# VitorMPCastro/MessyerRaytracer

Hardware: AMD Instinct MI355X
Metric: Mrays/s (primary, closest-hit) (higher is better)
Workload: dtype f32

## Files before the change

### messyerraytracer_amd/csrc/kernels.hip

```cpp
#include <hip/hip_runtime.h>
#include <cfloat>
#include <cstdarg>
#include <cstdio>
#include <cstdlib>
#include <type_traits>
#include "mrt_internal.h"

namespace mrt {

#define MRT_WG 256
#define MRT_WAVE 64

__device__ __forceinline__ float fma_(float a, float b, float c) { return __builtin_fmaf(a, b, c); }
__device__ __forceinline__ float dot3(float ax, float ay, float az, float bx, float by, float bz)
{
	return fma_(ax, bx, fma_(ay, by, az * bz));
}
__device__ __forceinline__ float safe_inv(float d)
{
	const float eps = 1e-9f;
	const float big = 1.0f / eps;
	return __builtin_fabsf(d) > eps ? 1.0f / d : (d >= 0.0f ? big : -big);
}

struct RayRegs {
	float ox, oy, oz, dx, dy, dz, t_min, t_max;
};

__device__ __forceinline__ bool skip_launch(const TraceParams &p)
{
	return p.skip_flag != nullptr && *p.skip_flag == p.skip_when;
}

__device__ __forceinline__ bool lane_ray_index_g(const TraceParams &p, uint64_t g, uint64_t &ray_idx, uint32_t &px, uint32_t &py);
__device__ __forceinline__ bool lane_ray_index(const TraceParams &p, uint32_t block, uint64_t &ray_idx, uint32_t &px, uint32_t &py)
{
	return lane_ray_index_g(p, (uint64_t)block * MRT_WG + threadIdx.x, ray_idx, px, py);
}
__device__ __forceinline__ bool xcd_strips(const TraceParams &p, uint64_t tile, uint32_t tiles_x, uint32_t tiles_y, uint32_t &tx, uint32_t &ty)
{
	const uint32_t tg = p.tile_group ? p.tile_group : 1u;
	uint32_t m = (tiles_x + 128u) >> 8;
	if (m == 0u) m = 1u;
	const uint32_t S = tiles_x / (8u * m);
	if (S == 0u || S * 8u * m != tiles_x || S % tg != 0u) return false;
	const uint64_t wg = tile / tg;
	const uint32_t k = (uint32_t)wg & 7u;
	const uint64_t j = (wg >> 3) * tg + tile % tg;
	const uint64_t per_strip = (uint64_t)S * tiles_y;
	const uint32_t sl = (uint32_t)(j / per_strip), r = (uint32_t)(j % per_strip);
	ty = r / S;
	tx = (sl * 8u + k) * S + r % S;
	return true;
}

__device__ __forceinline__ bool lane_ray_index_g(const TraceParams &p, uint64_t g, uint64_t &ray_idx, uint32_t &px, uint32_t &py)
{
	uint32_t lane_map = p.lane_map, grid_w = p.grid_w, rows = p.rows, tiles_x = p.tiles_x;
	if (lane_map == MAP_AUTO) {
		const uint32_t w = p.auto_grid[0];
		lane_map = w ? MAP_TILE8X8 : MAP_LINEAR;
		grid_w = w; rows = p.auto_grid[1]; tiles_x = p.auto_grid[2];
	}
	if (lane_map == MAP_TILE8X8) {
		uint64_t tile = g >> 6;
		const uint32_t l = (uint32_t)g & 63u;
		uint32_t tx, ty;
		const uint32_t k = p.tile_w_log2;
		const uint32_t tiles_y = (rows + (64u >> k) - 1u) >> (6u - k);
		uint32_t quarter = 4u;
		uint32_t sixteenth = 16u;
		if (p.quarter_all == 2u) { sixteenth = (uint32_t)tile & 15u; tile >>= 4; if (l >= 4u || tile >= (uint64_t)tiles_x * tiles_y) return false; }
		else if (p.quarter_all) { quarter = (uint32_t)tile & 3u; tile >>= 2; if (l >= 16u || tile >= (uint64_t)tiles_x * tiles_y) return false; }
		else if (p.tile_sched != nullptr && ((uint64_t)tiles_x * tiles_y + p.tile_unit - 1u) / p.tile_unit == p.n_units) {
			const uint64_t slot = tile / p.tile_unit;
			if (slot >= (p.sched_hdr ? p.sched_hdr[2] : p.n_units)) return false;
			const uint32_t e = p.tile_sched[slot], what = e >> 28, id = e & 0x0FFFFFFFu;
			if (what == 0u) tile = (uint64_t)id * p.tile_unit + tile % p.tile_unit;
			else {
				if (tile % p.tile_unit != 0u) return false;
				tile = id;
				if (what >= 2u) { quarter = what - 2u; if (l >= 16u) return false; }
			}
		}
		if (p.tile_order == 1u && (tiles_x & 15u) == 0u && (tiles_y & 15u) == 0u) {
			const uint32_t st = (uint32_t)(tile >> 8), in = (uint32_t)tile & 255u;
			uint32_t mx = in & 0x55u, my = (in >> 1) & 0x55u;
			mx = (mx | (mx >> 1)) & 0x33u; mx = (mx | (mx >> 2)) & 0x0Fu;
			my = (my | (my >> 1)) & 0x33u; my = (my | (my >> 2)) & 0x0Fu;
			const uint32_t stx = st % (tiles_x >> 4), sty = st / (tiles_x >> 4);
			tx = (stx << 4) + mx; ty = (sty << 4) + my;
		} else if (p.tile_order == 2u && (tiles_x & 31u) == 0u && (tiles_y & 31u) == 0u) {
			const uint32_t st = (uint32_t)(tile >> 10), in = (uint32_t)tile & 1023u;
			uint32_t mx = in & 0x155u, my = (in >> 1) & 0x155u;
			mx = (mx | (mx >> 1)) & 0x133u; mx = (mx | (mx >> 2)) & 0x10Fu; mx = (mx | (mx >> 4)) & 0x1Fu;
			my = (my | (my >> 1)) & 0x133u; my = (my | (my >> 2)) & 0x10Fu; my = (my | (my >> 4)) & 0x1Fu;
			const uint32_t stx = st % (tiles_x >> 5), sty = st / (tiles_x >> 5);
			tx = (stx << 5) + mx; ty = (sty << 5) + my;
		} else if (p.tile_order == 3u && xcd_strips(p, tile, tiles_x, tiles_y, tx, ty)) {
		} else { tx = (uint32_t)(tile % tiles_x); ty = (uint32_t)(tile / tiles_x); }
		if (sixteenth < 16u) {
			px = (tx << 3) + ((sixteenth & 3u) << 1) + (l & 1u);
			py = (ty << 3) + ((sixteenth >> 2) << 1) + (l >> 1);
		} else if (quarter < 4u) {
			px = (tx << 3) + ((quarter & 1u) << 2) + (l & 3u);
			py = (ty << 3) + ((quarter >> 1) << 2) + (l >> 2);
		} else {
			px = (tx << k) + (l & ((1u << k) - 1u));
			py = (ty << (6u - k)) + (l >> k);
		}
		if (px >= grid_w || py >= rows) return false;
		ray_idx = (uint64_t)py * grid_w + px;
		return true;
	}
	if (p.sparse_lanes) { const uint32_t l = (uint32_t)g & 63u; if (l >= p.sparse_lanes) return false; g = (g >> 6) * p.sparse_lanes + l; }
	if (g >= p.count) return false;
	ray_idx = p.perm ? (uint64_t)p.perm[g] : g;
	if (p.in_fmt == IN_GRID) { px = (uint32_t)(ray_idx % p.grid_w); py = (uint32_t)(ray_idx / p.grid_w); }
	return true;
}

__device__ __forceinline__ bool tile_cost_word(const TraceParams &p, uint64_t g_first, uint32_t *&park, uint32_t *&sum, uint32_t &what)
{
	if (p.tile_cost == nullptr) return false;
	uint32_t rows = p.rows, tiles_x = p.tiles_x;
	if (p.lane_map == MAP_AUTO) { if (p.auto_grid[0] == 0u) return false; rows = p.auto_grid[1]; tiles_x = p.auto_grid[2]; }
	else if (p.lane_map != MAP_TILE8X8) return false;
	const uint32_t k = p.tile_w_log2, tiles_y = (rows + (64u >> k) - 1u) >> (6u - k);
	if (((uint64_t)tiles_x * tiles_y + p.tile_unit - 1u) / p.tile_unit != p.n_units) return false;
	const uint64_t slot = (g_first >> 6) / p.tile_unit;
	what = 0u;
	if (p.tile_sched == nullptr) { if (slot >= p.n_units) return false; park = sum = p.tile_cost + slot; return true; }
	if (slot >= (p.sched_hdr ? p.sched_hdr[2] : p.n_units)) return false;
	const uint32_t e = p.tile_sched[slot], id = e & 0x0FFFFFFFu;
	what = e >> 28;
	if (what == 0u) { park = sum = p.tile_cost + id; return true; }
	park = p.tile_cost + p.n_units + slot;
	sum = p.tile_cost + id / p.tile_unit;
	return true;
}
__device__ __forceinline__ void note_tile_start(const TraceParams &p, uint64_t g_first)
{
	uint32_t *park, *sum, what;
	if (tile_cost_word(p, g_first, park, sum, what)) *park = (uint32_t)__builtin_amdgcn_s_memtime();
}
__device__ __forceinline__ void note_tile_cost(const TraceParams &p, uint64_t g_first)
{
	uint32_t *park, *sum, what;
	if (!tile_cost_word(p, g_first, park, sum, what)) return;
	uint32_t d = (uint32_t)__builtin_amdgcn_s_memtime() - *park;
	if (park == sum) { *sum = d ? d : 1u; return; }
	if (what == 1u) d = d - (d >> 2);
	else d = p.tile_unit == 2u ? (d >> 1) + (d >> 3) + (d >> 4) : d - (d >> 3);
	atomicAdd(sum, d ? d : 1u);
}

__device__ __forceinline__ void grid_ray(const TraceParams &p, uint32_t px, uint32_t py, RayRegs &r)
{
	const mrt_camera &c = p.cam;
	float dx, dy, dz;
	r.ox = c.origin[0]; r.oy = c.origin[1]; r.oz = c.origin[2];
	if (c.kind == MRT_CAMERA_DEBUG_GRID) {
		const float u = (2.0f * ((float)px + 0.5f) / (float)p.grid_w - 1.0f) * c.half_w;
		const float v = (2.0f * ((float)(py + p.y0) + 0.5f) / (float)p.grid_h - 1.0f) * c.half_h;
		dx = c.fwd[0] + c.right[0] * u + c.up[0] * v;
		dy = c.fwd[1] + c.right[1] * u + c.up[1] * v;
		dz = c.fwd[2] + c.right[2] * u + c.up[2] * v;
	} else {
		const float u = (2.0f * ((float)px + c.jitter_x) * c.inv_w) - 1.0f;
		const float v = 1.0f - (2.0f * ((float)(py + p.y0) + c.jitter_y) * c.inv_h);
		if (c.kind == MRT_CAMERA_PERSPECTIVE) {
			const float vx = u * c.half_w, vy = v * c.half_h;
			dx = c.right[0] * vx + c.up[0] * vy + c.fwd[0] * -1.0f;
			dy = c.right[1] * vx + c.up[1] * vy + c.fwd[1] * -1.0f;
			dz = c.right[2] * vx + c.up[2] * vy + c.fwd[2] * -1.0f;
		} else {
			const float sv = v * c.half_h, su = u * c.half_w;
			r.ox = (c.origin[0] + c.up[0] * sv) + c.right[0] * su;
			r.oy = (c.origin[1] + c.up[1] * sv) + c.right[1] * su;
			r.oz = (c.origin[2] + c.up[2] * sv) + c.right[2] * su;
			r.dx = -c.fwd[0]; r.dy = -c.fwd[1]; r.dz = -c.fwd[2];
			r.t_min = c.t_min; r.t_max = c.t_max;
			return;
		}
	}
	const float l2 = dx * dx + dy * dy + dz * dz;
	if (l2 == 0.0f) { dx = dy = dz = 0.0f; }
	else { const float l = __builtin_sqrtf(l2); dx /= l; dy /= l; dz /= l; }
	r.dx = dx; r.dy = dy; r.dz = dz;
	r.t_min = c.t_min; r.t_max = c.t_max;
}

__device__ __forceinline__ void load_ray(const TraceParams &p, uint64_t idx, uint32_t px, uint32_t py, RayRegs &r)
{
	if (p.in_fmt == IN_GRID) { grid_ray(p, px, py, r); return; }
	float ox, oy, oz, dx, dy, dz, t0, t1;
	if (p.in_fmt == IN_HOST60) {
		const float *h = reinterpret_cast<const float *>(p.rays) + idx * 15u;
		ox = h[0]; oy = h[1]; oz = h[2]; dx = h[3]; dy = h[4]; dz = h[5];
		t0 = h[12]; t1 = h[13];
	} else {
		const float4 *q = reinterpret_cast<const float4 *>(p.rays) + idx * 2u;
		const float4 a = q[0], b = q[1];
		ox = a.x; oy = a.y; oz = a.z; t1 = a.w;
		dx = b.x; dy = b.y; dz = b.z; t0 = b.w;
	}
	r.ox = ox; r.oy = oy; r.oz = oz; r.dx = dx; r.dy = dy; r.dz = dz; r.t_min = t0; r.t_max = t1;
}

__device__ __forceinline__ void store_hit(const TraceParams &p, uint64_t idx, const RayRegs &r,
		float t, int32_t prim, float u, float v, float nx, float ny, float nz, uint32_t layers, uint32_t slot)
{
	if (p.out_fmt == OUT_BOOL8) { reinterpret_cast<uint8_t *>(p.hits)[idx] = prim >= 0 ? 1 : 0; return; }
	if (p.out_fmt == OUT_TOKEN4) { reinterpret_cast<uint32_t *>(p.hits)[idx] = prim >= 0 ? slot : 0xFFFFFFFFu; return; }
	if (p.out_fmt == OUT_HOST44) {
		float *h = reinterpret_cast<float *>(p.hits) + idx * 11u;
		uint32_t *hu = reinterpret_cast<uint32_t *>(h);
		if (prim >= 0) {
			h[0] = t;
			h[1] = r.ox + r.dx * t; h[2] = r.oy + r.dy * t; h[3] = r.oz + r.dz * t;
			h[4] = nx; h[5] = ny; h[6] = nz; h[7] = u; h[8] = v;
			hu[9] = (uint32_t)prim; hu[10] = layers;
		} else {
			h[0] = FLT_MAX; h[1] = h[2] = h[3] = 0.0f; h[4] = h[5] = h[6] = 0.0f; h[7] = h[8] = 0.0f;
			hu[9] = 0xFFFFFFFFu; hu[10] = 0u;
		}
		return;
	}
	float4 *q = reinterpret_cast<float4 *>(p.hits) + idx * 2u;
	float4 a, b;
	a.x = t; a.y = __int_as_float(prim); a.z = u; a.w = v;
	b.x = nx; b.y = ny; b.z = nz; b.w = __uint_as_float(layers);
	q[0] = a; q[1] = b;
}

__device__ __forceinline__ void finish_ray(const TraceParams &p, uint64_t ray_idx, const RayRegs &r,
		float best_t, float best_u, float best_v, uint32_t best_slot)
{
	int32_t prim = -1; float nx = 0.0f, ny = 0.0f, nz = 0.0f; uint32_t layers = 0u;
	if (best_slot != 0xFFFFFFFFu) {
		if (p.out_fmt == OUT_BOOL8 || p.out_fmt == OUT_TOKEN4) prim = 0;
		else {
			prim = (int32_t)p.tri_hot[best_slot].id;
			layers = p.tri_hot[best_slot].layers;
			const float4 nn = reinterpret_cast<const float4 *>(p.tri_cold)[best_slot];
			nx = nn.x; ny = nn.y; nz = nn.z;
		}
	}
	store_hit(p, ray_idx, r, best_t, prim, best_u, best_v, nx, ny, nz, layers, best_slot);
}

__device__ __forceinline__ void finish_two_level_ray(const TraceParams &p, uint64_t ray_idx, const RayRegs &r,
		float best_t, float best_u, float best_v, uint32_t best_slot, uint32_t best_id, uint32_t best_inst)
{
	int32_t prim = -1; float nx = 0.0f, ny = 0.0f, nz = 0.0f; uint32_t layers = 0u;
	if (p.out_fmt == OUT_TOKEN8) {
		reinterpret_cast<uint2 *>(p.hits)[ray_idx] = make_uint2(best_slot, best_slot != 0xFFFFFFFFu ? best_inst : 0u);
		return;
	}
	if (best_slot != 0xFFFFFFFFu) {
		prim = (int32_t)best_id;
		if (p.out_fmt != OUT_BOOL8) {
			const float4 *row = reinterpret_cast<const float4 *>(p.instances) + (size_t)best_inst * 8u;
			const float4 b0 = row[3], b1 = row[4], b2 = row[5];
			const float4 no = reinterpret_cast<const float4 *>(p.tri_cold)[best_slot];
			nx = fma_(b0.x, no.x, fma_(b0.y, no.y, b0.z * no.z));
			ny = fma_(b0.w, no.x, fma_(b1.x, no.y, b1.y * no.z));
			nz = fma_(b1.z, no.x, fma_(b1.w, no.y, b2.x * no.z));
			const float l2 = fma_(nx, nx, fma_(ny, ny, nz * nz));
			if (l2 == 0.0f) { nx = ny = nz = 0.0f; }
			else { const float l = __builtin_sqrtf(l2); nx /= l; ny /= l; nz /= l; }
			layers = __float_as_uint(b2.w);
		}
	}
	store_hit(p, ray_idx, r, best_t, prim, best_u, best_v, nx, ny, nz, layers, best_slot);
}

#include "source_common.h"
#include "shadow_kernel.h"
#include "reflection_kernel.h"
#include "hemisphere_kernel.h"
#include "bounce_kernel.h"

template <bool ANY_HIT, bool COUNT>
__global__ __launch_bounds__(MRT_WG) void trace_lane_kernel(const TraceParams p)
{
	constexpr int SRC = SRC_CAST;
	const NoSource s{};
#include "lane_walk.inc"
}

#include "lane_persistent_kernel.h"
#include "packet_kernel.h"
#include "packet_asm_kernel.h"
#include "packet_rows_kernel.h"
#ifdef MRT_WITH_QUAD
#include "packet_quad_kernel.h"
#endif
#include "two_level_kernel.h"

template <class S, int SRC, bool ANY_HIT>
__global__ __launch_bounds__(MRT_WG) void trace_source_lane_kernel(const TraceParams p, const S s)
{
	constexpr bool COUNT = false;
#include "lane_walk.inc"
}
template <class S, int SRC, bool ANY_HIT>
__global__ __launch_bounds__(MRT_WG) void trace_source_two_level_kernel(const TraceParams p, const S s)
{
#include "two_level_walk.inc"
}
template <class S, int SRC, bool ANY_HIT, int WIDTH, bool TL>
__global__ __launch_bounds__(MRT_WG) MRT_PERSIST_ATTR void trace_source_persistent_kernel(const TraceParams p, const PersistParams q, const S s)
{
	constexpr bool COUNT = false;
#include "persistent_walk.inc"
}

__global__ __launch_bounds__(MRT_WG) void build_rows_kernel(const DevNode *nodes, const TriHot *hot, const TriCold *cold,
		uint32_t n_nodes, uint32_t n_tris, float4 *rows)
{
	const uint64_t g = (uint64_t)blockIdx.x * MRT_WG + threadIdx.x;
	if (g >= (uint64_t)n_nodes + n_tris) return;
	float4 *out = rows + g * 4u;
	if (g < n_nodes) {
		const float4 *n = reinterpret_cast<const float4 *>(nodes) + g * 4u;
		float4 a = n[0], b = n[1];
		uint32_t l = __float_as_uint(a.w), r = __float_as_uint(b.w);
		if (l >= kLeafBit) l = kLeafBit | (n_nodes + (l & 0x7FFFFFFFu));
		if (r >= kLeafBit) r = kLeafBit | (n_nodes + (r & 0x7FFFFFFFu));
		a.w = __uint_as_float(l); b.w = __uint_as_float(r);
		out[0] = a; out[1] = b; out[2] = n[2]; out[3] = n[3];
	} else {
		const uint64_t s = g - n_nodes;
		const float4 *t = reinterpret_cast<const float4 *>(hot) + s * 3u;
		out[0] = t[0]; out[1] = t[1]; out[2] = t[2];
		out[3] = reinterpret_cast<const float4 *>(cold)[s];
	}
}

hipError_t launch_build_rows(const DevNode *nodes, const TriHot *hot, const TriCold *cold, uint32_t n_nodes, uint32_t n_tris,
		void *rows, hipStream_t stream)
{
	const uint64_t total = (uint64_t)n_nodes + n_tris;
	hipLaunchKernelGGL(build_rows_kernel, dim3((uint32_t)((total + MRT_WG - 1) / MRT_WG)), dim3(MRT_WG), 0, stream,
			nodes, hot, cold, n_nodes, n_tris, reinterpret_cast<float4 *>(rows));
	return hipGetLastError();
}

__global__ __launch_bounds__(MRT_WG) void build_rows4_kernel(const Dev4Node *nodes4, const TriHot *hot, const TriCold *cold,
		uint32_t n_nodes4, uint32_t n_tris, float4 *rows)
{
	const uint64_t g = (uint64_t)blockIdx.x * MRT_WG + threadIdx.x;
	if (g >= (uint64_t)n_nodes4 + n_tris) return;
	if (g < n_nodes4) {
		const Dev4Node &n = nodes4[g];
		float *out = reinterpret_cast<float *>(rows + g * 8u);
		for (int k = 0; k < 4; k++)
			for (int c = 0; c < 3; c++) { out[6 * k + 2 * c] = n.box[k][c]; out[6 * k + 2 * c + 1] = n.box[k][3 + c]; }
		uint32_t *oref = reinterpret_cast<uint32_t *>(out) + 24;
		for (int i = 0; i < 4; i++) {
			const uint32_t ref = n.ref[i];
			oref[i] = ref == kSentinel ? ref : (ref >= kLeafBit ? (kLeafBit | (2u * n_nodes4 + (ref & 0x7FFFFFFFu))) : 2u * ref);
		}
		oref[4] = n.n_children; oref[5] = 0u; oref[6] = 0u; oref[7] = 0u;
	} else {
		const uint64_t s = g - n_nodes4;
		float4 *out = rows + ((uint64_t)2u * n_nodes4 + s) * 4u;
		const float4 *t = reinterpret_cast<const float4 *>(hot) + s * 3u;
		out[0] = t[0]; out[1] = t[1]; out[2] = t[2];
		out[3] = reinterpret_cast<const float4 *>(cold)[s];
	}
}

hipError_t launch_build_rows4(const Dev4Node *nodes4, const TriHot *hot, const TriCold *cold, uint32_t n_nodes4, uint32_t n_tris,
		void *rows, hipStream_t stream)
{
	const uint64_t total = (uint64_t)n_nodes4 + n_tris;
	hipLaunchKernelGGL(build_rows4_kernel, dim3((uint32_t)((total + MRT_WG - 1) / MRT_WG)), dim3(MRT_WG), 0, stream,
			nodes4, hot, cold, n_nodes4, n_tris, reinterpret_cast<float4 *>(rows));
	return hipGetLastError();
}

__global__ __launch_bounds__(MRT_WG) void grid_rays_kernel(const TraceParams p, mrt_ray32 *out)
{
	const uint64_t g = (uint64_t)blockIdx.x * MRT_WG + threadIdx.x;
	if (g >= p.count) return;
	RayRegs r;
	grid_ray(p, (uint32_t)(g % p.grid_w), (uint32_t)(g / p.grid_w), r);
	float4 *q = reinterpret_cast<float4 *>(out) + g * 2u;
	float4 a, b;
	a.x = r.ox; a.y = r.oy; a.z = r.oz; a.w = r.t_max;
	b.x = r.dx; b.y = r.dy; b.z = r.dz; b.w = r.t_min;
	q[0] = a; q[1] = b;
}

__global__ __launch_bounds__(MRT_WG) void expand_tokens_kernel(const TraceParams p, const uint32_t *tokens)
{
	const uint64_t g = (uint64_t)blockIdx.x * MRT_WG + threadIdx.x;
	if (g >= p.count) return;
	RayRegs r;
	uint32_t px = 0, py = 0;
	if (p.in_fmt == IN_GRID) { px = (uint32_t)(g % p.grid_w); py = (uint32_t)(g / p.grid_w); }
	load_ray(p, g, px, py, r);
	const uint32_t slot = tokens[g];
	if (slot >= p.n_tris) {
		store_hit(p, g, r, r.t_max, -1, 0.0f, 0.0f, 0.0f, 0.0f, 0.0f, 0u, slot);
		return;
	}
	const float4 *t3 = reinterpret_cast<const float4 *>(p.tri_hot) + (size_t)slot * 3u;
	const float4 q0 = t3[0], q1 = t3[1], q2 = t3[2];
	const float pvx = fma_(r.dy, q2.z, -(r.dz * q2.y));
	const float pvy = fma_(r.dz, q2.x, -(r.dx * q2.z));
	const float pvz = fma_(r.dx, q2.y, -(r.dy * q2.x));
	const float det = dot3(q1.x, q1.y, q1.z, pvx, pvy, pvz);
	const float inv_det = 1.0f / det;
	const float tvx = r.ox - q0.x, tvy = r.oy - q0.y, tvz = r.oz - q0.z;
	const float u = dot3(tvx, tvy, tvz, pvx, pvy, pvz) * inv_det;
	const float qvx = fma_(tvy, q1.z, -(tvz * q1.y));
	const float qvy = fma_(tvz, q1.x, -(tvx * q1.z));
	const float qvz = fma_(tvx, q1.y, -(tvy * q1.x));
	const float v = dot3(r.dx, r.dy, r.dz, qvx, qvy, qvz) * inv_det;
	const float t = dot3(q2.x, q2.y, q2.z, qvx, qvy, qvz) * inv_det;
	const float4 nn = reinterpret_cast<const float4 *>(p.tri_cold)[slot];
	store_hit(p, g, r, t, (int32_t)__float_as_uint(q0.w), u, v, nn.x, nn.y, nn.z, __float_as_uint(q1.w), slot);
}

__global__ __launch_bounds__(MRT_WG) void expand_two_level_tokens_kernel(const TraceParams p, const uint2 *tokens)
{
	const uint64_t g = (uint64_t)blockIdx.x * MRT_WG + threadIdx.x;
	if (g >= p.count) return;
	RayRegs r;
	uint32_t px = 0, py = 0;
	if (p.in_fmt == IN_GRID) { px = (uint32_t)(g % p.grid_w); py = (uint32_t)(g / p.grid_w); }
	load_ray(p, g, px, py, r);
	const uint2 tok = tokens[g];
	const uint32_t slot = tok.x, inst = tok.y;
	if (slot >= p.n_tris || inst >= p.n_instances) {
		finish_two_level_ray(p, g, r, r.t_max, 0.0f, 0.0f, 0xFFFFFFFFu, 0xFFFFFFFFu, 0u);
		return;
	}
	const float4 *row = reinterpret_cast<const float4 *>(p.instances) + (size_t)inst * 8u;
	const float4 m0 = row[0], m1 = row[1], m2 = row[2], meta = row[5];
	const float ox = fma_(m0.x, r.ox, fma_(m0.y, r.oy, fma_(m0.z, r.oz, m0.w)));
	const float oy = fma_(m1.x, r.ox, fma_(m1.y, r.oy, fma_(m1.z, r.oz, m1.w)));
	const float oz = fma_(m2.x, r.ox, fma_(m2.y, r.oy, fma_(m2.z, r.oz, m2.w)));
	const float dx = fma_(m0.x, r.dx, fma_(m0.y, r.dy, m0.z * r.dz));
	const float dy = fma_(m1.x, r.dx, fma_(m1.y, r.dy, m1.z * r.dz));
	const float dz = fma_(m2.x, r.dx, fma_(m2.y, r.dy, m2.z * r.dz));
	const float4 *t3 = reinterpret_cast<const float4 *>(p.tri_hot) + (size_t)slot * 3u;
	const float4 q0 = t3[0], q1 = t3[1], q2 = t3[2];
	const float pvx = fma_(dy, q2.z, -(dz * q2.y));
	const float pvy = fma_(dz, q2.x, -(dx * q2.z));
	const float pvz = fma_(dx, q2.y, -(dy * q2.x));
	const float det = dot3(q1.x, q1.y, q1.z, pvx, pvy, pvz);
	const float inv_det = 1.0f / det;
	const float tvx = ox - q0.x, tvy = oy - q0.y, tvz = oz - q0.z;
	const float u = dot3(tvx, tvy, tvz, pvx, pvy, pvz) * inv_det;
	const float qvx = fma_(tvy, q1.z, -(tvz * q1.y));
	const float qvy = fma_(tvz, q1.x, -(tvx * q1.z));
	const float qvz = fma_(tvx, q1.y, -(tvy * q1.x));
	const float v = dot3(dx, dy, dz, qvx, qvy, qvz) * inv_det;
	const float t = dot3(q2.x, q2.y, q2.z, qvx, qvy, qvz) * inv_det;
	finish_two_level_ray(p, g, r, t, u, v, slot, __float_as_uint(meta.z) + __float_as_uint(q0.w), inst);
}

#define MRT_DETECT_THREADS 1024
#define MRT_DETECT_MAX_RAYS 65536u
__device__ __forceinline__ void ray_dir(const void *rays, uint32_t in_fmt, uint64_t i, float &x, float &y, float &z)
{
	if (in_fmt == IN_HOST60) {
		const float *h = reinterpret_cast<const float *>(rays) + i * 15u;
		x = h[3]; y = h[4]; z = h[5];
	} else {
		const float4 b = reinterpret_cast<const float4 *>(rays)[i * 2u + 1u];
		x = b.x; y = b.y; z = b.z;
	}
}
__global__ __launch_bounds__(MRT_DETECT_THREADS) void detect_grid_kernel(const void *rays, uint32_t in_fmt, uint64_t count,
		uint32_t tile_w_log2, unsigned long long *scratch, uint32_t *out, uint32_t *host_out)
{
	__shared__ uint32_t first, second, is_last;
	const uint32_t m = (uint32_t)(count < (uint64_t)MRT_DETECT_MAX_RAYS ? count : (uint64_t)MRT_DETECT_MAX_RAYS);
	float ax, ay, az, bx, by, bz;
	ray_dir(rays, in_fmt, 0, ax, ay, az);
	ray_dir(rays, in_fmt, 1, bx, by, bz);
	const float step2 = (bx - ax) * (bx - ax) + (by - ay) * (by - ay) + (bz - az) * (bz - az);
	const float thr = 36.0f * step2;
	const uint32_t i = blockIdx.x * MRT_DETECT_THREADS + threadIdx.x;
	bool jump = false, wide = false;
	if (i >= 1 && i < m) {
		ray_dir(rays, in_fmt, i - 1, ax, ay, az);
		ray_dir(rays, in_fmt, i, bx, by, bz);
		const float d2 = (bx - ax) * (bx - ax) + (by - ay) * (by - ay) + (bz - az) * (bz - az);
		jump = d2 > thr;
		wide = !(d2 <= 0.01f);
	}
	const unsigned long long mask = __ballot(jump);
	const unsigned long long wmask_dir = __ballot(wide);
	if ((threadIdx.x & 63u) == 0u) {
		__hip_atomic_store(&scratch[i >> 6], mask, __ATOMIC_RELAXED, __HIP_MEMORY_SCOPE_AGENT);
		if (wmask_dir) atomicAdd(&scratch[1025], (unsigned long long)__builtin_popcountll(wmask_dir));
	}
	__threadfence();
	__syncthreads();
	if (threadIdx.x == 0) {
		const unsigned long long t = atomicAdd(&scratch[1024], 1ull);
		is_last = (t == (unsigned long long)gridDim.x - 1ull) ? 1u : 0u;
		first = 0xFFFFFFFFu; second = 0xFFFFFFFFu;
	}
	__syncthreads();
	if (!is_last) return;
	__threadfence();
	const uint32_t words = (m + 63u) >> 6;
	unsigned long long wmask = 0ull;
	if (threadIdx.x < words) wmask = __hip_atomic_load(&scratch[threadIdx.x], __ATOMIC_RELAXED, __HIP_MEMORY_SCOPE_AGENT);
	if (wmask) atomicMin(&first, threadIdx.x * 64u + (uint32_t)__builtin_ctzll(wmask));
	__syncthreads();
	const uint32_t f = first;
	if (f != 0xFFFFFFFFu && threadIdx.x >= (f >> 6)) {
		unsigned long long rest = wmask;
		if (threadIdx.x == (f >> 6)) rest &= ~((2ull << (f & 63u)) - 1ull);
		if (rest) atomicMin(&second, threadIdx.x * 64u + (uint32_t)__builtin_ctzll(rest));
	}
	__syncthreads();
	if (threadIdx.x == 0) {
		uint32_t w = first, rows = 0, tiles_x = 0;
		const uint32_t tw = 1u << tile_w_log2, th = 64u >> tile_w_log2;
		bool ok = step2 > 0.0f && w != 0xFFFFFFFFu && w >= 16u && (w % tw) == 0u && (count % w) == 0ull;
		if (ok) {
			const uint64_t r = count / w;
			ok = r <= 0xFFFFFFFFull && (r % th) == 0ull && (2ull * w >= m || second == 2u * w);
			rows = (uint32_t)r; tiles_x = w >> tile_w_log2;
		}
		out[0] = ok ? w : 0u; out[1] = ok ? rows : 0u; out[2] = ok ? tiles_x : 0u;
		const unsigned long long n_wide = __hip_atomic_load(&scratch[1025], __ATOMIC_RELAXED, __HIP_MEMORY_SCOPE_AGENT);
		out[3] = (n_wide * 8ull > (unsigned long long)m || (!ok && count < 32768ull)) ? 1u : 0u;
		if (host_out) { host_out[0] = out[0]; host_out[1] = out[1]; host_out[2] = out[2]; host_out[3] = out[3]; }
		scratch[1024] = 0ull; scratch[1025] = 0ull;
	}
}

hipError_t launch_detect_grid(const void *rays, uint32_t in_fmt, uint64_t count, uint32_t tile_w_log2,
		unsigned long long *scratch, uint32_t *out, uint32_t *host_out, hipStream_t stream)
{
	const uint32_t m = (uint32_t)(count < (uint64_t)MRT_DETECT_MAX_RAYS ? count : (uint64_t)MRT_DETECT_MAX_RAYS);
	const uint32_t blocks = (m + MRT_DETECT_THREADS - 1) / MRT_DETECT_THREADS;
	hipLaunchKernelGGL(detect_grid_kernel, dim3(blocks), dim3(MRT_DETECT_THREADS), 0, stream, rays, in_fmt, count, tile_w_log2, scratch, out, host_out);
	return hipGetLastError();
}

__device__ __forceinline__ uint32_t spread10(uint32_t v)
{
	v &= 0x000003FFu;
	v = (v | (v << 16)) & 0x030000FFu;
	v = (v | (v << 8)) & 0x0300F00Fu;
	v = (v | (v << 4)) & 0x030C30C3u;
	v = (v | (v << 2)) & 0x09249249u;
	return v;
}
__device__ __forceinline__ uint32_t quant10(float v)
{
	float n = (v + 1.0f) * 0.5f;
	n = fmaxf(0.0f, fminf(1.0f, n));
	return (uint32_t)(n * 1023.0f);
}
__global__ __launch_bounds__(MRT_WG) void morton_keys_kernel(const void *rays, uint32_t in_fmt, uint64_t count,
		uint32_t *keys, uint32_t *index)
{
	const uint64_t g = (uint64_t)blockIdx.x * MRT_WG + threadIdx.x;
	if (g >= count) return;
	float dx, dy, dz;
	if (in_fmt == IN_HOST60) {
		const float *h = reinterpret_cast<const float *>(rays) + g * 15u;
		dx = h[3]; dy = h[4]; dz = h[5];
	} else {
		const float4 b = reinterpret_cast<const float4 *>(rays)[g * 2u + 1u];
		dx = b.x; dy = b.y; dz = b.z;
	}
	keys[g] = (spread10(quant10(dx)) << 2) | (spread10(quant10(dy)) << 1) | spread10(quant10(dz));
	if (index) index[g] = (uint32_t)g;
}

__global__ __launch_bounds__(MRT_WG) void origin_dir_keys_kernel(const void *rays, uint32_t in_fmt, uint64_t count,
		float bx, float by, float bz, float sx, float sy, float sz, uint32_t *keys, uint32_t *index)
{
	const uint64_t g = (uint64_t)blockIdx.x * MRT_WG + threadIdx.x;
	if (g >= count) return;
	float ox, oy, oz, dx, dy, dz;
	if (in_fmt == IN_HOST60) {
		const float *h = reinterpret_cast<const float *>(rays) + g * 15u;
		ox = h[0]; oy = h[1]; oz = h[2]; dx = h[3]; dy = h[4]; dz = h[5];
	} else {
		const float4 a = reinterpret_cast<const float4 *>(rays)[g * 2u], b = reinterpret_cast<const float4 *>(rays)[g * 2u + 1u];
		ox = a.x; oy = a.y; oz = a.z; dx = b.x; dy = b.y; dz = b.z;
	}
	auto q = [](float v, float lo, float scale, float top) {
		const float n = fmaxf(0.0f, fminf(top, (v - lo) * scale));
		return (uint32_t)n;
	};
	const uint32_t qx = q(ox, bx, sx, 63.0f), qy = q(oy, by, sy, 63.0f), qz = q(oz, bz, sz, 63.0f);
	const uint32_t ex = q(dx, -1.0f, 8.0f, 15.0f), ey = q(dy, -1.0f, 8.0f, 15.0f), ez = q(dz, -1.0f, 8.0f, 15.0f);
	const uint32_t ko = (spread10(qx) << 2) | (spread10(qy) << 1) | spread10(qz);
	const uint32_t kd = (spread10(ex) << 2) | (spread10(ey) << 1) | spread10(ez);
	keys[g] = (ko << 12) | kd;
	if (index) index[g] = (uint32_t)g;
}

hipError_t launch_origin_dir_keys(const void *rays, uint32_t in_fmt, uint64_t count, const float lo[3], const float hi[3],
		uint32_t *keys, uint32_t *index, hipStream_t stream)
{
	if (count == 0) return hipSuccess;
	const uint64_t blocks = (count + MRT_WG - 1) / MRT_WG;
	float s[3];
	for (int k = 0; k < 3; k++) { const float e = hi[k] - lo[k]; s[k] = e > 0.0f ? 64.0f / e : 0.0f; }
	hipLaunchKernelGGL(origin_dir_keys_kernel, dim3((uint32_t)blocks), dim3(MRT_WG), 0, stream, rays, in_fmt, count,
			lo[0], lo[1], lo[2], s[0], s[1], s[2], keys, index);
	return hipGetLastError();
}

bool quad_kernel_built()
{
#ifdef MRT_WITH_QUAD
	return true;
#else
	return false;
#endif
}
static thread_local char g_variant[96] = "";
const char *last_trace_variant() { return g_variant; }
static void note_variant(const char *fmt, ...)
{
	va_list ap; va_start(ap, fmt); vsnprintf(g_variant, sizeof(g_variant), fmt, ap); va_end(ap);
}
#define MRT_B(x) ((x) ? "true" : "false")
#ifndef MRT_ROWS_WG_LARGE
#define MRT_ROWS_WG_LARGE MRT_WG
#endif
constexpr uint32_t kPrefetchMaxWaves = kWaveSlots + kWaveSlots / 4u;
hipError_t launch_trace(const TraceParams &p_in, bool any_hit, bool count, hipStream_t stream)
{
	TraceParams p = p_in;
	p.tile_group = (p.kernel == MRT_KERNEL_PACKET_DUAL && p.row_array != nullptr) ? 2u * ((p.rows_wg == 64u ? 64u : (uint32_t)MRT_ROWS_WG_LARGE) / MRT_WAVE) : MRT_WG / MRT_WAVE;
	uint64_t threads;
	if (p.tile_sched != nullptr && p.sched_hdr != nullptr && p.n_slots_max != 0u) {
		threads = (uint64_t)p.n_slots_max * p.tile_unit * 64u;
		if (p.lane_map == MAP_AUTO && threads < p.count) threads = p.count;
	} else if (p.lane_map == MAP_TILE8X8) {
		const uint32_t th = 64u >> p.tile_w_log2;
		threads = (uint64_t)p.tiles_x * ((p.rows + th - 1u) / th) * 64u * (p.quarter_all == 2u ? 16u : (p.quarter_all ? 4u : 1u));
	} else if (p.lane_map == MAP_LINEAR && p.sparse_lanes) threads = (p.count + p.sparse_lanes - 1u) / p.sparse_lanes * 64u;
	else threads = p.count * ((p.lane_map == MAP_AUTO && p.quarter_all) ? (p.quarter_all == 2u ? 16u : 4u) : 1u);
	if (threads == 0) return hipSuccess;
	const uint64_t blocks = (threads + MRT_WG - 1) / MRT_WG;
	if (blocks > 0x7FFFFFFFull) return hipErrorInvalidValue;
	dim3 grid((uint32_t)blocks), wg(MRT_WG);
	if (p.kernel == MRT_KERNEL_TWO_LEVEL_PACKET) {
		if (any_hit) hipLaunchKernelGGL((trace_two_level_packet_kernel<true>), grid, wg, p.extra_lds, stream, p);
		else hipLaunchKernelGGL((trace_two_level_packet_kernel<false>), grid, wg, p.extra_lds, stream, p);
		note_variant("trace_two_level_packet_kernel<%s>", MRT_B(any_hit));
		return hipGetLastError();
	}
	if (p.kernel == MRT_KERNEL_TWO_LEVEL) {
		const size_t lds2 = (size_t)(MRT_WG / MRT_WAVE) * p.stack_depth * MRT_WAVE * sizeof(uint32_t);
		if (any_hit) hipLaunchKernelGGL((trace_two_level_kernel<true>), grid, wg, lds2, stream, p);
		else hipLaunchKernelGGL((trace_two_level_kernel<false>), grid, wg, lds2, stream, p);
		note_variant("trace_two_level_kernel<%s>", MRT_B(any_hit));
		return hipGetLastError();
	}
#ifdef MRT_WITH_QUAD
	if (p.kernel == MRT_KERNEL_PACKET_QUAD && p.row_array4 != nullptr) {
		const uint64_t rblocks = (threads + 2u * MRT_WG - 1) / (2u * MRT_WG);
		dim3 rgrid((uint32_t)rblocks);
		if (count) {
			if (any_hit) hipLaunchKernelGGL((trace_packet_quad_kernel<true, true>), rgrid, wg, p.extra_lds, stream, p);
			else hipLaunchKernelGGL((trace_packet_quad_kernel<false, true>), rgrid, wg, p.extra_lds, stream, p);
		} else if (any_hit) hipLaunchKernelGGL((trace_packet_quad_kernel<true, false>), rgrid, wg, p.extra_lds, stream, p);
		else hipLaunchKernelGGL((trace_packet_quad_kernel<false, false>), rgrid, wg, p.extra_lds, stream, p);
		note_variant("trace_packet_quad_kernel<%s, %s>", MRT_B(any_hit), MRT_B(count));
		return hipGetLastError();
	}
#endif
	if ((p.kernel == MRT_KERNEL_PACKET_DUAL || p.kernel == MRT_KERNEL_PACKET_ROWS) && p.row_array != nullptr) {
		const uint32_t packets = p.kernel == MRT_KERNEL_PACKET_DUAL ? 2u : 1u;
		const uint32_t rows_wg = packets == 2u && p.rows_wg == 64u ? 64u : (packets == 2u ? (uint32_t)MRT_ROWS_WG_LARGE : (uint32_t)MRT_WG);
		const uint64_t rblocks = (threads + packets * rows_wg - 1) / (packets * rows_wg);
		dim3 rgrid((uint32_t)rblocks), rwg(rows_wg);
#define MRT_LAUNCH_ROWS(A, C, N, W, F) hipLaunchKernelGGL((trace_packet_rows_kernel<A, C, N, W, F>), rgrid, rwg, p.extra_lds, stream, p)
#define MRT_LAUNCH_ROWS_AC(N, W, F)                                                                                    \
		do {                                                                                                        \
			if (count) { if (any_hit) MRT_LAUNCH_ROWS(true, true, N, W, F); else MRT_LAUNCH_ROWS(false, true, N, W, F); } \
			else { if (any_hit) MRT_LAUNCH_ROWS(true, false, N, W, F); else MRT_LAUNCH_ROWS(false, false, N, W, F); }   \
		} while (0)
		const bool cull = packets == 2u && (p.rows_cull == 1u || (p.rows_cull == 2u && p.in_fmt == IN_GRID));
		if (packets == 2u && rows_wg == 64u) { if (cull) MRT_LAUNCH_ROWS_AC(2, 64, true); else MRT_LAUNCH_ROWS_AC(2, 64, false); }
		else if (packets == 2u) { if (cull) MRT_LAUNCH_ROWS_AC(2, MRT_ROWS_WG_LARGE, true); else MRT_LAUNCH_ROWS_AC(2, MRT_ROWS_WG_LARGE, false); }
		else MRT_LAUNCH_ROWS_AC(1, MRT_WG, false);
#undef MRT_LAUNCH_ROWS_AC
#undef MRT_LAUNCH_ROWS
		note_variant("trace_packet_rows_kernel<%s, %s, %u, %u, %s>", MRT_B(any_hit), MRT_B(count), packets, rows_wg, MRT_B(cull));
		return hipGetLastError();
	}
	if ((p.kernel == MRT_KERNEL_PACKET_ASM || p.kernel == MRT_KERNEL_PACKET_DUAL || p.kernel == MRT_KERNEL_PACKET_ROWS || p.kernel == MRT_KERNEL_PACKET_QUAD) && p.n_nodes < kAsmNodeLimit) {
		if (count) {
			if (any_hit) hipLaunchKernelGGL((trace_packet_asm_kernel<true, true>), grid, wg, p.extra_lds, stream, p);
			else hipLaunchKernelGGL((trace_packet_asm_kernel<false, true>), grid, wg, p.extra_lds, stream, p);
		} else {
			uint64_t waves = p.tile_sched != nullptr && p.n_slots_max != 0u ? (p.n_units > kWaveSlots ? p.n_units : (p.n_slots_max < kWaveSlots ? p.n_slots_max : kWaveSlots)) : threads / MRT_WAVE;
			if (p.lane_map == MAP_AUTO && waves < (p.count + MRT_WAVE - 1u) / MRT_WAVE) waves = (p.count + MRT_WAVE - 1u) / MRT_WAVE;
			const bool kpf = waves <= kPrefetchMaxWaves;
			if (kpf) { if (any_hit) hipLaunchKernelGGL((trace_packet_asm_kernel<true, false, true>), grid, wg, p.extra_lds, stream, p);
				else hipLaunchKernelGGL((trace_packet_asm_kernel<false, false, true>), grid, wg, p.extra_lds, stream, p); }
			else if (any_hit) hipLaunchKernelGGL((trace_packet_asm_kernel<true>), grid, wg, p.extra_lds, stream, p);
			else hipLaunchKernelGGL((trace_packet_asm_kernel<false>), grid, wg, p.extra_lds, stream, p);
			if (kpf) { note_variant("trace_packet_asm_kernel<%s, false, true>", MRT_B(any_hit)); return hipGetLastError(); }
		}
		note_variant("trace_packet_asm_kernel<%s, %s>", MRT_B(any_hit), MRT_B(count));
		return hipGetLastError();
	}
	if (p.kernel == MRT_KERNEL_PACKET || p.kernel == MRT_KERNEL_PACKET_ASM || p.kernel == MRT_KERNEL_PACKET_DUAL || p.kernel == MRT_KERNEL_PACKET_ROWS || p.kernel == MRT_KERNEL_PACKET_QUAD) {
		if (any_hit) {
			if (count) hipLaunchKernelGGL((trace_packet_kernel<true, true>), grid, wg, 0, stream, p);
			else hipLaunchKernelGGL((trace_packet_kernel<true, false>), grid, wg, 0, stream, p);
		} else {
			if (count) hipLaunchKernelGGL((trace_packet_kernel<false, true>), grid, wg, 0, stream, p);
			else hipLaunchKernelGGL((trace_packet_kernel<false, false>), grid, wg, 0, stream, p);
		}
		note_variant("trace_packet_kernel<%s, %s>", MRT_B(any_hit), MRT_B(count));
		return hipGetLastError();
	}
	const size_t lds = (size_t)(MRT_WG / MRT_WAVE) * p.stack_depth * MRT_WAVE * sizeof(uint32_t);
	if (any_hit) {
		if (count) hipLaunchKernelGGL((trace_lane_kernel<true, true>), grid, wg, lds, stream, p);
		else hipLaunchKernelGGL((trace_lane_kernel<true, false>), grid, wg, lds, stream, p);
	} else {
		if (count) hipLaunchKernelGGL((trace_lane_kernel<false, true>), grid, wg, lds, stream, p);
		else hipLaunchKernelGGL((trace_lane_kernel<false, false>), grid, wg, lds, stream, p);
	}
	note_variant("trace_lane_kernel<%s, %s>", MRT_B(any_hit), MRT_B(count));
	return hipGetLastError();
}

static PersistParams persist_params(const TraceParams &p, unsigned long long *next_ray, uint32_t *overflow,
		uint32_t lds_depth, uint32_t refill, uint32_t leaf_wait, uint32_t blocks)
{
	PersistParams q;
	q.next_ray = next_ray; q.overflow = overflow; q.overflow_stride = blocks * MRT_WG;
	q.lds_depth = lds_depth; q.refill = refill; q.leaf_wait = leaf_wait ? leaf_wait : 1u;
	const uint64_t per_wave = p.count / ((uint64_t)blocks * (MRT_WG / MRT_WAVE)) / 32u;
	q.chunk = per_wave >= MRT_RAY_CHUNK ? MRT_RAY_CHUNK : (per_wave <= MRT_WAVE ? MRT_WAVE : (uint32_t)(per_wave & ~63ull));
	return q;
}

hipError_t launch_trace_persistent(const TraceParams &p, unsigned long long *next_ray, uint32_t *overflow,
		uint32_t lds_depth, uint32_t refill, uint32_t leaf_wait, uint32_t blocks, bool any_hit, bool count, hipStream_t stream)
{
	if (p.count == 0 || blocks == 0) return hipSuccess;
	const PersistParams q = persist_params(p, next_ray, overflow, lds_depth, refill, leaf_wait, blocks);
	const size_t lds = (size_t)(MRT_WG / MRT_WAVE) * lds_depth * MRT_WAVE * sizeof(uint32_t);
	const bool wide8 = p.kernel == MRT_KERNEL_LANE8_PERSISTENT && p.nodes8 != nullptr;
	const bool wide4 = p.kernel == MRT_KERNEL_LANE4_PERSISTENT && p.nodes4 != nullptr;
	if (p.kernel == MRT_KERNEL_TWO_LEVEL_PERSISTENT8 && p.nodes8 != nullptr && p.leaf_box != nullptr) {
		if (any_hit) hipLaunchKernelGGL((trace_lane_persistent_kernel<true, 8, true>), dim3(blocks), dim3(MRT_WG), lds, stream, p, q);
		else hipLaunchKernelGGL((trace_lane_persistent_kernel<false, 8, true>), dim3(blocks), dim3(MRT_WG), lds, stream, p, q);
	} else if (p.kernel == MRT_KERNEL_TWO_LEVEL_PERSISTENT || p.kernel == MRT_KERNEL_TWO_LEVEL_PERSISTENT8) {
		if (any_hit) hipLaunchKernelGGL((trace_lane_persistent_kernel<true, 2, true>), dim3(blocks), dim3(MRT_WG), lds, stream, p, q);
		else hipLaunchKernelGGL((trace_lane_persistent_kernel<false, 2, true>), dim3(blocks), dim3(MRT_WG), lds, stream, p, q);
	} else if (count) {
#define MRT_LP(A, W) hipLaunchKernelGGL((trace_lane_persistent_kernel<A, W, false, true>), dim3(blocks), dim3(MRT_WG), lds, stream, p, q)
		if (wide8) { if (any_hit) MRT_LP(true, 8); else MRT_LP(false, 8); }
		else if (wide4) { if (any_hit) MRT_LP(true, 4); else MRT_LP(false, 4); }
		else { if (any_hit) MRT_LP(true, 2); else MRT_LP(false, 2); }
#undef MRT_LP
	} else if (wide8) {
		if (any_hit) hipLaunchKernelGGL((trace_lane_persistent_kernel<true, 8>), dim3(blocks), dim3(MRT_WG), lds, stream, p, q);
		else hipLaunchKernelGGL((trace_lane_persistent_kernel<false, 8>), dim3(blocks), dim3(MRT_WG), lds, stream, p, q);
	} else if (wide4) {
		if (any_hit) hipLaunchKernelGGL((trace_lane_persistent_kernel<true, 4>), dim3(blocks), dim3(MRT_WG), lds, stream, p, q);
		else hipLaunchKernelGGL((trace_lane_persistent_kernel<false, 4>), dim3(blocks), dim3(MRT_WG), lds, stream, p, q);
	} else {
		if (any_hit) hipLaunchKernelGGL((trace_lane_persistent_kernel<true, 2>), dim3(blocks), dim3(MRT_WG), lds, stream, p, q);
		else hipLaunchKernelGGL((trace_lane_persistent_kernel<false, 2>), dim3(blocks), dim3(MRT_WG), lds, stream, p, q);
	}
	{
		const bool tl = p.kernel == MRT_KERNEL_TWO_LEVEL_PERSISTENT || p.kernel == MRT_KERNEL_TWO_LEVEL_PERSISTENT8;
		const int width = tl ? ((p.kernel == MRT_KERNEL_TWO_LEVEL_PERSISTENT8 && p.nodes8 != nullptr && p.leaf_box != nullptr) ? 8 : 2) : (wide8 ? 8 : (wide4 ? 4 : 2));
		note_variant("trace_lane_persistent_kernel<%s, %d, %s, %s>", MRT_B(any_hit), width, MRT_B(tl), MRT_B(count && !tl));
	}
	return hipGetLastError();
}

template <class S, int SRC, bool ANY_HIT>
static void launch_source_as(const TraceParams &p, const S &s, unsigned long long *next_ray, uint32_t *overflow,
		uint32_t lds_depth, uint32_t refill, uint32_t leaf_wait, uint32_t blocks, hipStream_t stream)
{
	using F = SourceFamily<S>;
	const bool tl = p.kernel == MRT_KERNEL_TWO_LEVEL || p.kernel == MRT_KERNEL_TWO_LEVEL_PERSISTENT || p.kernel == MRT_KERNEL_TWO_LEVEL_PERSISTENT8;
	char mode[8] = "";
	if (F::any_hit && F::nearest) snprintf(mode, sizeof(mode), ", %s", MRT_B(ANY_HIT));
	if (blocks == 0) {
		const uint64_t threads = p.sparse_lanes ? (p.count + p.sparse_lanes - 1u) / p.sparse_lanes * 64u : p.count;
		const dim3 grid((uint32_t)((threads + MRT_WG - 1) / MRT_WG)), wg(MRT_WG);
		const size_t lds = (size_t)(MRT_WG / MRT_WAVE) * p.stack_depth * MRT_WAVE * sizeof(uint32_t);
		if (tl) hipLaunchKernelGGL((trace_source_two_level_kernel<S, SRC, ANY_HIT>), grid, wg, lds, stream, p, s);
		else hipLaunchKernelGGL((trace_source_lane_kernel<S, SRC, ANY_HIT>), grid, wg, lds, stream, p, s);
		note_variant("trace_%s_%s_kernel<%d%s>", F::name, tl ? "two_level" : "lane", SRC, mode);
		return;
	}
	const PersistParams q = persist_params(p, next_ray, overflow, lds_depth, refill, leaf_wait, blocks);
	const size_t lds = (size_t)(MRT_WG / MRT_WAVE) * q.lds_depth * MRT_WAVE * sizeof(uint32_t);
#define MRT_LS(W, T) hipLaunchKernelGGL((trace_source_persistent_kernel<S, SRC, ANY_HIT, W, T>), dim3(blocks), dim3(MRT_WG), lds, stream, p, q, s)
	int width = 2;
	if (tl && p.kernel == MRT_KERNEL_TWO_LEVEL_PERSISTENT8 && p.nodes8 != nullptr && p.leaf_box != nullptr) { width = 8; MRT_LS(8, true); }
	else if (tl) MRT_LS(2, true);
	else if (p.kernel == MRT_KERNEL_LANE8_PERSISTENT && p.nodes8 != nullptr) { width = 8; MRT_LS(8, false); }
	else if (p.kernel == MRT_KERNEL_LANE4_PERSISTENT && p.nodes4 != nullptr) { width = 4; MRT_LS(4, false); }
	else MRT_LS(2, false);
#undef MRT_LS
	note_variant("trace_%s_persistent_kernel<%d%s, %d, %s>", F::name, SRC, mode, width, MRT_B(tl));
}

template <class S>
hipError_t launch_source(const TraceParams &p, const void *params, int src, bool any_hit, unsigned long long *next_ray, uint32_t *overflow,
		uint32_t lds_depth, uint32_t refill, uint32_t leaf_wait, uint32_t blocks, hipStream_t stream)
{
	using F = SourceFamily<S>;
	const S &s = *static_cast<const S *>(params);
	if (p.count == 0) return hipSuccess;
	const uint64_t threads = p.sparse_lanes ? (p.count + p.sparse_lanes - 1u) / p.sparse_lanes * 64u : p.count;
	if (blocks == 0 && (threads + MRT_WG - 1) / MRT_WG > 0x7FFFFFFFull) return hipErrorInvalidValue;
	if ((src != F::ray32 && src != F::host && src != F::grid) || !(any_hit ? F::any_hit : F::nearest)) return hipErrorInvalidValue;
#define MRT_LS_SRC(A)                                                                                                                        \
	do {                                                                                                                                 \
		if (src == F::ray32) launch_source_as<S, F::ray32, A>(p, s, next_ray, overflow, lds_depth, refill, leaf_wait, blocks, stream);   \
		else if (src == F::host) launch_source_as<S, F::host, A>(p, s, next_ray, overflow, lds_depth, refill, leaf_wait, blocks, stream); \
		else launch_source_as<S, F::grid, A>(p, s, next_ray, overflow, lds_depth, refill, leaf_wait, blocks, stream);                     \
	} while (0)
	if constexpr (F::any_hit) { if (any_hit) MRT_LS_SRC(true); }
	if constexpr (F::nearest) { if (!any_hit) MRT_LS_SRC(false); }
#undef MRT_LS_SRC
	return hipGetLastError();
}
template hipError_t launch_source<ShadowParams>(const TraceParams &, const void *, int, bool, unsigned long long *, uint32_t *, uint32_t, uint32_t, uint32_t, uint32_t, hipStream_t);
template hipError_t launch_source<ReflectParams>(const TraceParams &, const void *, int, bool, unsigned long long *, uint32_t *, uint32_t, uint32_t, uint32_t, uint32_t, hipStream_t);
template hipError_t launch_source<HemiParams>(const TraceParams &, const void *, int, bool, unsigned long long *, uint32_t *, uint32_t, uint32_t, uint32_t, uint32_t, hipStream_t);
template hipError_t launch_source<BounceParams>(const TraceParams &, const void *, int, bool, unsigned long long *, uint32_t *, uint32_t, uint32_t, uint32_t, uint32_t, hipStream_t);

hipError_t launch_grid_rays(const TraceParams &p, mrt_ray32 *out, hipStream_t stream)
{
	if (p.count == 0) return hipSuccess;
	const uint64_t blocks = (p.count + MRT_WG - 1) / MRT_WG;
	hipLaunchKernelGGL(grid_rays_kernel, dim3((uint32_t)blocks), dim3(MRT_WG), 0, stream, p, out);
	return hipGetLastError();
}

hipError_t launch_expand_tokens(const TraceParams &p, const uint32_t *tokens, hipStream_t stream)
{
	if (p.count == 0) return hipSuccess;
	const uint64_t blocks = (p.count + MRT_WG - 1) / MRT_WG;
	if (p.instances != nullptr)
		hipLaunchKernelGGL(expand_two_level_tokens_kernel, dim3((uint32_t)blocks), dim3(MRT_WG), 0, stream, p, reinterpret_cast<const uint2 *>(tokens));
	else hipLaunchKernelGGL(expand_tokens_kernel, dim3((uint32_t)blocks), dim3(MRT_WG), 0, stream, p, tokens);
	return hipGetLastError();
}

hipError_t launch_morton_keys(const void *rays, uint32_t in_fmt, uint64_t count, uint32_t *keys, uint32_t *index, hipStream_t stream)
{
	if (count == 0) return hipSuccess;
	const uint64_t blocks = (count + MRT_WG - 1) / MRT_WG;
	hipLaunchKernelGGL(morton_keys_kernel, dim3((uint32_t)blocks), dim3(MRT_WG), 0, stream, rays, in_fmt, count, keys, index);
	return hipGetLastError();
}

}
```

### messyerraytracer_amd/csrc/packet_rows_kernel.h

```cpp
#pragma once

#define RA_LMINX "s20"
#define RA_LMINY "s21"
#define RA_LMINZ "s22"
#define RA_LREF "s23"
#define RA_LMAXX "s24"
#define RA_LMAXY "s25"
#define RA_LMAXZ "s26"
#define RA_RREF "s27"
#define RA_RMINX "s28"
#define RA_RMINY "s29"
#define RA_RMINZ "s30"
#define RA_RMAXX "s32"
#define RA_RMAXY "s33"
#define RA_RMAXZ "s34"
#define RA_MASK "s[60:61]"
#define RA_MASKLO "s60"
#define RA_MASKHI "s61"
#define RA_V0X "s20"
#define RA_V0Y "s21"
#define RA_V0Z "s22"
#define RA_ID "s23"
#define RA_E1X "s24"
#define RA_E1Y "s25"
#define RA_E1Z "s26"
#define RA_LAYERS "s27"
#define RA_E2X "s28"
#define RA_E2Y "s29"
#define RA_E2Z "s30"
#define RA_FLAGS "s31"

#define MRT_NEAR_0(RS, AX, SIDE) RS##_##SIDE##MIN##AX
#define MRT_NEAR_1(RS, AX, SIDE) RS##_##SIDE##MAX##AX
#define MRT_FAR_0(RS, AX, SIDE) RS##_##SIDE##MAX##AX
#define MRT_FAR_1(RS, AX, SIDE) RS##_##SIDE##MIN##AX

#define MRT_OP(NAME, P) "%[" NAME P "]"

#define MRT_ROWS_SLAB(P, RS, BX, BY, BZ)                                                                             \
	"v_fma_f32 v50, " MRT_NEAR_##BX(RS, X, L) ", " MRT_OP("ix", P) ", " MRT_OP("nrx", P) "\n"                        \
	"v_fma_f32 v51, " MRT_NEAR_##BY(RS, Y, L) ", " MRT_OP("iy", P) ", " MRT_OP("nry", P) "\n"                        \
	"v_fma_f32 v52, " MRT_NEAR_##BZ(RS, Z, L) ", " MRT_OP("iz", P) ", " MRT_OP("nrz", P) "\n"                        \
	"v_fma_f32 v53, " MRT_FAR_##BX(RS, X, L) ", " MRT_OP("ix", P) ", " MRT_OP("nrx", P) "\n"                         \
	"v_fma_f32 v54, " MRT_FAR_##BY(RS, Y, L) ", " MRT_OP("iy", P) ", " MRT_OP("nry", P) "\n"                         \
	"v_fma_f32 v55, " MRT_FAR_##BZ(RS, Z, L) ", " MRT_OP("iz", P) ", " MRT_OP("nrz", P) "\n"                         \
	"v_max_f32 v52, v52, " MRT_OP("tmin", P) "\n"                                                                   \
	"v_fma_f32 v56, " MRT_NEAR_##BX(RS, X, R) ", " MRT_OP("ix", P) ", " MRT_OP("nrx", P) "\n"                        \
	"v_min_f32 v55, v55, " MRT_OP("lim", P) "\n"                                                                    \
	"v_fma_f32 v57, " MRT_NEAR_##BY(RS, Y, R) ", " MRT_OP("iy", P) ", " MRT_OP("nry", P) "\n"                        \
	"v_max3_f32 v50, v50, v51, v52\n"                                                               \
	"v_fma_f32 v51, " MRT_NEAR_##BZ(RS, Z, R) ", " MRT_OP("iz", P) ", " MRT_OP("nrz", P) "\n"                        \
	"v_min3_f32 v53, v53, v54, v55\n"                                                               \
	"v_fma_f32 v52, " MRT_FAR_##BX(RS, X, R) ", " MRT_OP("ix", P) ", " MRT_OP("nrx", P) "\n"                         \
	"v_fma_f32 v54, " MRT_FAR_##BY(RS, Y, R) ", " MRT_OP("iy", P) ", " MRT_OP("nry", P) "\n"                         \
	"v_fma_f32 v55, " MRT_FAR_##BZ(RS, Z, R) ", " MRT_OP("iz", P) ", " MRT_OP("nrz", P) "\n"                         \
	"v_max_f32 v51, v51, " MRT_OP("tmin", P) "\n"                                                                   \
	"v_min_f32 v55, v55, " MRT_OP("lim", P) "\n"                                                                    \
	"v_max3_f32 v56, v56, v57, v51\n"                                                               \
	"v_min3_f32 v52, v52, v54, v55\n"

#define MRT_ROWS_NODE_STEP(P, RS, POPBIT, CNT_P, BX, BY, BZ)                                                                 \
	MRT_ROWS_SLAB(P, RS, BX, BY, BZ)                                                                                \
	"v_cmp_le_f32 vcc, v50, v53\n"                                             \
	"v_cmp_le_f32_e64 s[54:55], v56, v52\n"                                    \
	"s_cbranch_vccz L_" P "lmiss_%=\n"                                                                              \
	"s_cmp_eq_u64 s[54:55], 0\n"                                                                                    \
	"s_cbranch_scc1 L_" P "onlyl_%=\n"                                                                              \
	"v_cmp_lt_f32_e64 s[56:57], v50, v56\n"     \
	"s_bitcmp1_b32 s56, 0\n"                                                                                        \
	"s_cselect_b32 s53, " RS##_RREF ", " RS##_LREF "\n"                                                    \
	"s_cselect_b32 " MRT_OP("cur", P) ", " RS##_LREF ", " RS##_RREF "\n"                                   \
	"s_cselect_b64 s[58:59], s[54:55], vcc\n"                                   \
	"s_cselect_b64 " RS##_MASK ", vcc, s[54:55]\n"                               \
	"v_mov_b32 v51, s53\n"                                                                                          \
	"v_mov_b32 v52, s58\n"                                                                                          \
	"v_mov_b32 v53, s59\n"                                                                                          \
	"ds_write_b32 " MRT_OP("sp", P) ", v51\n"                                                                       \
	"ds_write_b64 " MRT_OP("sp", P) ", v[52:53] offset:8\n"                                                         \
	"v_add_u32 " MRT_OP("sp", P) ", 16, " MRT_OP("sp", P) "\n"                                                      \
	CNT_P                                                                                                           \
	"v_lshlrev_b32 v54, 6, v51\n"             \
	"global_load_dword v60, v54, %[rows]\n"   \
	"s_branch L_" P "done_%=\n"                                                                                     \
	"L_" P "onlyl_%=:\n"                                                                                            \
	"s_mov_b32 " MRT_OP("cur", P) ", " RS##_LREF "\n"                                                                \
	"s_mov_b64 " RS##_MASK ", vcc\n"                                                                                 \
	"s_branch L_" P "done_%=\n"                                                                                     \
	"L_" P "lmiss_%=:\n"                                                                                            \
	"s_cmp_eq_u64 s[54:55], 0\n"                                                                                    \
	"s_cbranch_scc1 L_" P "npop_%=\n"                                                                               \
	"s_mov_b32 " MRT_OP("cur", P) ", " RS##_RREF "\n"                                                                \
	"s_mov_b64 " RS##_MASK ", s[54:55]\n"                                                                            \
	"s_branch L_" P "done_%=\n"                                                                                     \
	"L_" P "npop_%=:\n"                                                                                             \
	"s_or_b32 %[ev], %[ev], " POPBIT "\n"

#define MRT_ROWS_TRI_TEST(P, RS, OWNMASK, CUROP, ANYHIT_CODE)                                                        \
	"s_and_b32 s52, " RS##_LAYERS ", %[qmask]\n"                    \
	"s_cbranch_scc0 L_" P "tnext_%=\n"                                                                              \
	"v_mul_f32 v50, " RS##_E2Y ", " MRT_OP("dz", P) "\n"                                                             \
	"v_mul_f32 v51, " RS##_E2Z ", " MRT_OP("dx", P) "\n"                                                             \
	"v_mul_f32 v52, " RS##_E2X ", " MRT_OP("dy", P) "\n"                                                             \
	"v_fma_f32 v50, " MRT_OP("dy", P) ", " RS##_E2Z ", -v50\n"                            \
	"v_fma_f32 v51, " MRT_OP("dz", P) ", " RS##_E2X ", -v51\n"                            \
	"v_fma_f32 v52, " MRT_OP("dx", P) ", " RS##_E2Y ", -v52\n"                            \
	"v_mul_f32 v53, " RS##_E1Z ", v52\n"                                                                             \
	"v_fma_f32 v53, " RS##_E1Y ", v51, v53\n"                                                                        \
	"v_fma_f32 v53, " RS##_E1X ", v50, v53\n"                                                     \
	"v_cmp_nlt_f32_e64 s[54:55], |v53|, %[eps]\n"                                              \
	"s_and_b64 s[54:55], s[54:55], " OWNMASK "\n"                       \
	"s_cbranch_scc0 L_" P "tnext_%=\n"                                                                              \
	"v_div_scale_f32 v54, s[56:57], v53, v53, 1.0\n"                   \
	"v_rcp_f32 v55, v54\n"                                                                                          \
	"v_div_scale_f32 v56, vcc, 1.0, v53, 1.0\n"                                                                     \
	"v_subrev_f32 v59, " RS##_V0X ", " MRT_OP("ox", P) "\n"       \
	"v_fma_f32 v57, -v54, v55, 1.0\n"                                                                               \
	"v_fma_f32 v55, v57, v55, v55\n"                                                                                \
	"v_mul_f32 v57, v56, v55\n"                                                                                     \
	"v_fma_f32 v58, -v54, v57, v56\n"                                                                               \
	"v_fma_f32 v57, v58, v55, v57\n"                                                                                \
	"v_fma_f32 v54, -v54, v57, v56\n"                                                                               \
	"v_div_fmas_f32 v54, v54, v55, v57\n"                                                                           \
	"v_div_fixup_f32 v54, v54, v53, 1.0\n"                                                       \
	"v_subrev_f32 v55, " RS##_V0Y ", " MRT_OP("oy", P) "\n"                                                 \
	"v_subrev_f32 v56, " RS##_V0Z ", " MRT_OP("oz", P) "\n"                                                 \
	"v_mul_f32 v58, v56, v52\n"                                                                                     \
	"v_fma_f32 v58, v55, v51, v58\n"                                                                                \
	"v_fma_f32 v58, v59, v50, v58\n"                                                                                \
	"v_mul_f32 v58, v58, v54\n"                                                    \
	"v_cmp_nlt_f32_e64 s[56:57], v58, 0\n"                                                            \
	"v_cmp_ngt_f32_e64 s[58:59], v58, 1.0\n"                                                          \
	"s_and_b64 s[54:55], s[54:55], s[56:57]\n"                                                                      \
	"s_and_b64 s[54:55], s[54:55], s[58:59]\n"                                                                      \
	"s_cbranch_scc0 L_" P "tnext_%=\n"                                                                              \
	"v_mul_f32 v50, " RS##_E1Y ", v56\n"                                                                             \
	"v_mul_f32 v51, " RS##_E1Z ", v59\n"                                                                             \
	"v_mul_f32 v52, " RS##_E1X ", v55\n"                                                                             \
	"v_fma_f32 v50, v55, " RS##_E1Z ", -v50\n"                                          \
	"v_fma_f32 v51, v56, " RS##_E1X ", -v51\n"                                          \
	"v_fma_f32 v52, v59, " RS##_E1Y ", -v52\n"                                          \
	"v_mul_f32 v59, " MRT_OP("dz", P) ", v52\n"                                                                     \
	"v_fma_f32 v59, " MRT_OP("dy", P) ", v51, v59\n"                                                                \
	"v_fma_f32 v59, " MRT_OP("dx", P) ", v50, v59\n"                                                                \
	"v_mul_f32 v59, v59, v54\n"                                                     \
	"v_add_f32 v55, v58, v59\n"                                                                          \
	"v_cmp_nlt_f32_e64 s[56:57], v59, 0\n"                                                            \
	"v_cmp_ngt_f32_e64 s[58:59], v55, 1.0\n"                                                      \
	"s_and_b64 s[54:55], s[54:55], s[56:57]\n"                                                                      \
	"s_and_b64 s[54:55], s[54:55], s[58:59]\n"                                                                      \
	"s_cbranch_scc0 L_" P "tnext_%=\n"                                                                              \
	"v_mul_f32 v55, " RS##_E2Z ", v52\n"                                                                             \
	"v_fma_f32 v55, " RS##_E2Y ", v51, v55\n"                                                                        \
	"v_fma_f32 v55, " RS##_E2X ", v50, v55\n"                                                                        \
	"v_mul_f32 v55, v55, v54\n"                                                    \
	                          \
	"v_cmp_nlt_f32_e64 s[56:57], v55, " MRT_OP("tmin", P) "\n"                                                      \
	"v_cmp_lt_f32_e64 s[58:59], v55, " MRT_OP("lim", P) "\n"                                                        \
	"v_cmp_eq_f32_e64 s[64:65], v55, " MRT_OP("lim", P) "\n"                                                        \
	"v_cmp_ne_u32_e64 s[66:67], " MRT_OP("bs", P) ", -1\n"                                                          \
	"v_cmp_gt_u32_e64 vcc, " MRT_OP("bi", P) ", " RS##_ID "\n"                                     \
	"s_and_b64 s[64:65], s[64:65], s[66:67]\n"                                                                      \
	"s_and_b64 s[64:65], s[64:65], vcc\n"                                                                           \
	"s_or_b64 s[58:59], s[58:59], s[64:65]\n"                                                                       \
	"s_and_b64 s[54:55], s[54:55], s[56:57]\n"                                                                      \
	"s_and_b64 s[54:55], s[54:55], s[58:59]\n"                                    \
	"s_cbranch_scc0 L_" P "tnext_%=\n"                                                                              \
	"s_and_b32 s52, " CUROP ", 0x7fffffff\n"                                                \
	"v_mov_b32 v50, s52\n"                                                                                          \
	"v_mov_b32 v51, " RS##_ID "\n"                                                                                   \
	"v_cndmask_b32_e64 " MRT_OP("bt", P) ", " MRT_OP("bt", P) ", v55, s[54:55]\n"                                   \
	"v_cndmask_b32_e64 " MRT_OP("bu", P) ", " MRT_OP("bu", P) ", v58, s[54:55]\n"                                   \
	"v_cndmask_b32_e64 " MRT_OP("bv", P) ", " MRT_OP("bv", P) ", v59, s[54:55]\n"                                   \
	"v_cndmask_b32_e64 " MRT_OP("bs", P) ", " MRT_OP("bs", P) ", v50, s[54:55]\n"                                   \
	"v_cndmask_b32_e64 " MRT_OP("bi", P) ", " MRT_OP("bi", P) ", v51, s[54:55]\n"                                   \
	ANYHIT_CODE                                                                                                     \
	"L_" P "tnext_%=:\n"

#define MRT_ROWS_TRI_STEP(P, RS, POPBIT, CNT_T, ANYHIT_CODE)                                                         \
	CNT_T                                                                                                           \
	MRT_ROWS_TRI_TEST(P, RS, RS##_MASK, MRT_OP("cur", P), ANYHIT_CODE)                                              \
	"s_bitcmp1_b32 " RS##_FLAGS ", 0\n"                                          \
	"s_cbranch_scc1 L_" P "tpop_%=\n"                                                                               \
	"s_add_u32 " MRT_OP("cur", P) ", " MRT_OP("cur", P) ", 1\n"                                                     \
	"s_branch L_" P "done_%=\n"                                                                                     \
	"L_" P "tpop_%=:\n"                                                                                             \
	"s_or_b32 %[ev], %[ev], " POPBIT "\n"

#define MRT_ROWS_NEAREST(P) \
	"v_cndmask_b32_e64 " MRT_OP("lim", P) ", " MRT_OP("lim", P) ", v55, s[54:55]\n"
#define MRT_ROWS_ANYHIT(P, DONEBIT) \
	"v_cndmask_b32_e64 " MRT_OP("lim", P) ", " MRT_OP("lim", P) ", %[vneg], s[54:55]\n"                             \
	"v_cmp_neq_f32_e64 s[56:57], " MRT_OP("lim", P) ", %[vneg]\n"                                                   \
	"s_cmp_lg_u64 s[56:57], 0\n"                                                                                    \
	"s_cbranch_scc1 L_" P "tnext_%=\n"                                                                              \
	"s_mov_b32 " MRT_OP("cur", P) ", 0x7fffffff\n"                                                                  \
	"s_or_b32 %[ev], %[ev], " DONEBIT "\n"                                                                          \
	"s_branch L_" P "done_%=\n"

#define MRT_ROWS_STEP(P, RS, POPBIT, CNT_N, CNT_T, CNT_P, ANYHIT_CODE, BX, BY, BZ)                                            \
	"s_bitcmp1_b32 " MRT_OP("cur", P) ", 31\n"                                                                      \
	"s_cbranch_scc1 L_" P "tri_%=\n"                                                                                \
	CNT_N                                                                                                           \
	MRT_ROWS_NODE_STEP(P, RS, POPBIT, CNT_P, BX, BY, BZ)                                                             \
	"s_branch L_" P "done_%=\n"                                                                                     \
	"L_" P "tri_%=:\n"                                                                                              \
	MRT_ROWS_TRI_STEP(P, RS, POPBIT, CNT_T, ANYHIT_CODE)                                                             \
	"L_" P "done_%=:\n"

#define MRT_ROWS_POP_ISSUE(P, POPBITNO, V0123)                                                                      \
	"s_bitcmp1_b32 %[ev], " POPBITNO "\n"                                                                           \
	"s_cbranch_scc0 L_" P "pi_%=\n"                                                                                 \
	"v_add_u32 " MRT_OP("sp", P) ", -16, " MRT_OP("sp", P) "\n"                                                     \
	"ds_read_b128 " V0123 ", " MRT_OP("sp", P) "\n"                                                                 \
	"L_" P "pi_%=:\n"
#define MRT_ROWS_POP_TAKE(P, RS, POPBITNO, V0, V2, V3)                                                               \
	"s_bitcmp1_b32 %[ev], " POPBITNO "\n"                                                                           \
	"s_cbranch_scc0 L_" P "pt_%=\n"                                                                                 \
	"v_readfirstlane_b32 " MRT_OP("cur", P) ", " V0 "\n"                                                            \
	"v_readfirstlane_b32 " RS##_MASKLO ", " V2 "\n"                                                                  \
	"v_readfirstlane_b32 " RS##_MASKHI ", " V3 "\n"                                                                  \
	"L_" P "pt_%=:\n"

#define MRT_ROWS_CLOBBERS                                                                                             \
	"vcc", "scc", "s20", "s21", "s22", "s23", "s24", "s25", "s26", "s27", "s28", "s29", "s30", "s31", "s32", "s33", \
	"s34", "s35", "s36", "s37", "s38", "s39", "s40", "s41", "s42", "s43", "s44", "s45", "s46", "s47", "s48", "s49", \
	"s50", "s51", "s52", "s53", "s54", "s55", "s56", "s57", "s58", "s59", "s60", "s61", "s62", "s63", "s64", "s65", \
	"s66", "s67", "v50", "v51", "v52", "v53", "v54", "v55", "v56", "v57", "v58", "v59", "v60"

#define MRT_ROWS_OUT(P, S)                                                                                            \
	[cur##P] "+s"(S.cur), [sp##P] "+v"(S.sp), [lim##P] "+v"(S.lim), [bt##P] "+v"(S.bt), [bu##P] "+v"(S.bu),         \
	[bv##P] "+v"(S.bv), [bs##P] "+v"(S.bs), [bi##P] "+v"(S.bi), [mask##P] "+s"(S.mask)
#define MRT_ROWS_IN(P, S)                                                                                             \
	[ox##P] "v"(S.ox), [oy##P] "v"(S.oy), [oz##P] "v"(S.oz), [dx##P] "v"(S.dx), [dy##P] "v"(S.dy), [dz##P] "v"(S.dz), \
	[tmin##P] "v"(S.tmin), [ix##P] "v"(S.ix), [iy##P] "v"(S.iy), [iz##P] "v"(S.iz), [nrx##P] "v"(S.nrx),            \
	[nry##P] "v"(S.nry), [nrz##P] "v"(S.nrz)

struct PacketRegs {
	float ox, oy, oz, dx, dy, dz, tmin;
	float ix, iy, iz, nrx, nry, nrz;
	float lim;
	float bt, bu, bv;
	uint32_t bs, bi;
	uint32_t sp;
	uint32_t cur;
	unsigned long long mask;
};

#define MRT_ROWS_LOOP1(CNT_N, CNT_T, CNT_P, T_PRE, T_POST, ANYHIT_CODE, BX, BY, BZ)                                          \
	asm volatile(                                                                                                   \
		"s_mov_b64 s[60:61], %[maskA]\n"                                                                            \
		"L_loop_%=:\n"                                                                                              \
		"s_lshl_b32 s52, %[curA], 6\n"                                                                              \
		T_PRE                                                                                                       \
		"s_load_dwordx16 s[20:35], %[rows], s52\n"                                                                  \
		"s_waitcnt lgkmcnt(0)\n"                                                                                    \
		T_POST                                                                                                      \
		MRT_ROWS_STEP("A", RA, "1", CNT_N, CNT_T, CNT_P, ANYHIT_CODE, BX, BY, BZ)                                   \
		"s_cmp_eq_u32 %[ev], 0\n"                                                                                   \
		"s_cbranch_scc1 L_loop_%=\n"                                                                                \
		MRT_ROWS_POP_ISSUE("A", "0", "v[50:53]")                                                                    \
		"s_waitcnt lgkmcnt(0)\n"                                                                                    \
		MRT_ROWS_POP_TAKE("A", RA, "0", "v50", "v52", "v53")                                                        \
		"s_mov_b32 %[ev], 0\n"                                                                                      \
		"s_cmp_lg_u32 %[curA], 0x7fffffff\n"                                                                        \
		"s_cbranch_scc1 L_loop_%=\n"                                                                                \
		"s_waitcnt vmcnt(0)\n"                    \
		"s_mov_b64 %[maskA], s[60:61]\n"                                                                            \
		: MRT_ROWS_OUT(A, a), [ev] "+s"(ev), [cntn] "+s"(cnt_n), [cntt] "+s"(cnt_t), [cntw] "+s"(cnt_w), [cntp] "+s"(sp_max) \
		: MRT_ROWS_IN(A, a), [rows] "s"(rows), [qmask] "s"(qmask), [eps] "s"(eps), [vneg] "v"(vneg)                 \
		: MRT_ROWS_CLOBBERS)

#define MRT_ROWSW_GROUP_SLAB(P, OWN, LM, RM, BX, BY, BZ)                                                              \
	"s_cmp_eq_u64 " OWN ", 0\n"                                                                                     \
	"s_cbranch_scc1 L_" P "skip_%=\n"                             \
	MRT_ROWS_SLAB(P, RA, BX, BY, BZ)                                                                                \
	"v_cmp_le_f32_e64 " LM ", v50, v53\n"                                                                           \
	"v_cmp_le_f32_e64 " RM ", v56, v52\n"                                                                           \
	"L_" P "sdone_%=:\n"
#define MRT_ROWSW_GROUP_SKIP(P, LM, RM)                                                                               \
	"L_" P "skip_%=:\n"                                                                                             \
	"s_mov_b64 " LM ", 0\n"                                                                                         \
	"s_mov_b64 " RM ", 0\n"                                                                                         \
	"s_branch L_" P "sdone_%=\n"

#define MRT_ROWSW_ANYHIT(P) \
	"v_cndmask_b32_e64 " MRT_OP("lim", P) ", " MRT_OP("lim", P) ", %[vneg], s[54:55]\n"
#define MRT_ROWSW_ANYDONE                                                                                             \
	"v_cmp_neq_f32_e64 s[56:57], %[limA], %[vneg]\n"                                                                \
	"v_cmp_neq_f32_e64 s[58:59], %[limB], %[vneg]\n"                                                                \
	"s_or_b64 s[56:57], s[56:57], s[58:59]\n"                                                                       \
	"s_cbranch_scc1 L_goon_%=\n"                                                                                    \
	"s_mov_b32 %[curA], 0x7fffffff\n"                                                                               \
	"s_branch L_exit_%=\n"                                                                                          \
	"L_goon_%=:\n"

#ifndef MRT_ROWS_KPREFETCH
#define MRT_ROWS_KPREFETCH 1
#endif
#if MRT_ROWS_KPREFETCH
#define MRT_ROWSW_KPREFETCH                                                                                           \
	"s_lshl_b32 s48, " RA_LREF ", 6\n"                                                                               \
	"s_lshl_b32 s49, " RA_RREF ", 6\n"                                                                               \
	"s_load_dword s64, %[rows], s48\n"                                                                              \
	"s_load_dword s65, %[rows], s49\n"
#define MRT_ROWSW_FARPREFETCH ""
#else
#define MRT_ROWSW_KPREFETCH ""
#define MRT_ROWSW_FARPREFETCH                                                                                         \
	"v_lshlrev_b32 v55, 6, v54\n"                                       \
	"global_load_dword v60, v55, %[rows]\n"
#endif

#define MRT_ROWS_LOOPW(CNT_N, CNT_T, CNT_P, ANYA, ANYB, ANYDONE, BX, BY, BZ)                                                 \
	asm volatile(                                                                                                   \
		"s_mov_b64 s[60:61], %[maskA]\n"                                                                            \
		"s_mov_b64 s[62:63], %[maskB]\n"                                                                            \
		"L_loop_%=:\n"                                                                                              \
		"s_lshl_b32 s52, %[curA], 6\n"                                                                              \
		"s_load_dwordx16 s[20:35], %[rows], s52\n"                                                                  \
		"s_waitcnt lgkmcnt(0)\n"                                                                                    \
		"s_bitcmp1_b32 %[curA], 31\n"                                                                               \
		"s_cbranch_scc1 L_tri_%=\n"                                                                                 \
		CNT_N                                                                                                       \
		MRT_ROWSW_KPREFETCH                                                                                         \
		MRT_ROWSW_GROUP_SLAB("A", "s[60:61]", "s[36:37]", "s[38:39]", BX, BY, BZ)                                   \
		MRT_ROWSW_GROUP_SLAB("B", "s[62:63]", "s[40:41]", "s[42:43]", BX, BY, BZ)                                   \
		"s_or_b64 s[44:45], s[36:37], s[40:41]\n"                     \
		"s_cbranch_scc0 L_lmiss_%=\n"                                                                               \
		"s_or_b64 vcc, s[38:39], s[42:43]\n"                                              \
		"s_cbranch_scc0 L_onlyl_%=\n"                                                                               \
		      \
		"v_cmp_lt_f32_e64 s[46:47], v50, v56\n"                                           \
		"s_bitcmp1_b32 s46, 0\n"                                                                                    \
		"s_cselect_b32 s53, " RA_RREF ", " RA_LREF "\n"                                                   \
		"s_cselect_b32 %[curA], " RA_LREF ", " RA_RREF "\n"                                               \
		"s_cselect_b64 s[50:51], s[38:39], s[36:37]\n"                 \
		"s_cselect_b64 s[58:59], s[42:43], s[40:41]\n"                                                              \
		"s_cselect_b64 s[60:61], s[36:37], s[38:39]\n"                                        \
		"s_cselect_b64 s[62:63], s[40:41], s[42:43]\n"                                                              \
		"v_mov_b32 v50, s50\n"                                                                                      \
		"v_mov_b32 v51, s51\n"                                                                                      \
		"v_mov_b32 v52, s58\n"                                                                                      \
		"v_mov_b32 v53, s59\n"                                                                                      \
		"v_mov_b32 v54, s53\n"                                                                                      \
		"ds_write_b128 %[spA], v[50:53]\n"                                                                          \
		"ds_write_b32 %[spA], v54 offset:16\n"                                                                      \
		"v_add_u32 %[spA], 32, %[spA]\n"                                                                            \
		CNT_P                                                                                                       \
		MRT_ROWSW_FARPREFETCH                                                                                       \
		"s_branch L_loop_%=\n"                                                                                      \
		"L_onlyl_%=:\n"                                                                                             \
		"s_mov_b32 %[curA], " RA_LREF "\n"                                                                          \
		"s_mov_b64 s[60:61], s[36:37]\n"                                                                            \
		"s_mov_b64 s[62:63], s[40:41]\n"                                                                            \
		"s_branch L_loop_%=\n"                                                                                      \
		"L_lmiss_%=:\n"                                                                                             \
		"s_or_b64 vcc, s[38:39], s[42:43]\n"                                                                        \
		"s_cbranch_scc0 L_pop_%=\n"                                                                                 \
		"s_mov_b32 %[curA], " RA_RREF "\n"                                                                          \
		"s_mov_b64 s[60:61], s[38:39]\n"                                                                            \
		"s_mov_b64 s[62:63], s[42:43]\n"                                                                            \
		"s_branch L_loop_%=\n"                                                                                      \
		"L_tri_%=:\n"                                                                                               \
		CNT_T                                                                                                       \
		"s_cmp_eq_u64 s[60:61], 0\n"                                                                                \
		"s_cbranch_scc1 L_Atnext_%=\n"                                                                              \
		MRT_ROWS_TRI_TEST("A", RA, "s[60:61]", "%[curA]", ANYA)                                                     \
		"s_cmp_eq_u64 s[62:63], 0\n"                                                                                \
		"s_cbranch_scc1 L_Btnext_%=\n"                                                                              \
		MRT_ROWS_TRI_TEST("B", RA, "s[62:63]", "%[curA]", ANYB)                                                     \
		ANYDONE                                                                                                     \
		"s_bitcmp1_b32 " RA_FLAGS ", 0\n"                                       \
		"s_cbranch_scc1 L_pop_%=\n"                                                                                 \
		"s_add_u32 %[curA], %[curA], 1\n"                                                                           \
		"s_branch L_loop_%=\n"                                                                                      \
		"L_pop_%=:\n"                                                                                               \
		"v_add_u32 %[spA], -32, %[spA]\n"                                                                           \
		"ds_read_b128 v[50:53], %[spA]\n"                                                                           \
		"ds_read_b32 v54, %[spA] offset:16\n"                                                                       \
		"s_waitcnt lgkmcnt(0)\n"                                                                                    \
		"v_readfirstlane_b32 %[curA], v54\n"                                                                        \
		"v_readfirstlane_b32 s60, v50\n"                                                                            \
		"v_readfirstlane_b32 s61, v51\n"                                                                            \
		"v_readfirstlane_b32 s62, v52\n"                                                                            \
		"v_readfirstlane_b32 s63, v53\n"                                                                            \
		"s_cmp_lg_u32 %[curA], 0x7fffffff\n"                                                                        \
		"s_cbranch_scc1 L_loop_%=\n"                                                                                \
		"s_branch L_exit_%=\n"                                                                                      \
		MRT_ROWSW_GROUP_SKIP("A", "s[36:37]", "s[38:39]")                                                           \
		MRT_ROWSW_GROUP_SKIP("B", "s[40:41]", "s[42:43]")                                                           \
		"L_exit_%=:\n"                                                                                              \
		"s_waitcnt vmcnt(0)\n"                    \
		"s_mov_b64 %[maskA], s[60:61]\n"                                                                            \
		"s_mov_b64 %[maskB], s[62:63]\n"                                                                            \
		: MRT_ROWS_OUT(A, a), [limB] "+v"(b.lim), [btB] "+v"(b.bt), [buB] "+v"(b.bu), [bvB] "+v"(b.bv),             \
		  [bsB] "+v"(b.bs), [biB] "+v"(b.bi), [maskB] "+s"(b.mask), [cntn] "+s"(cnt_n), [cntt] "+s"(cnt_t), [cntp] "+s"(sp_max) \
		: MRT_ROWS_IN(A, a), MRT_ROWS_IN(B, b), [rows] "s"(rows), [qmask] "s"(qmask), [eps] "s"(eps), [vneg] "v"(vneg) \
		: MRT_ROWS_CLOBBERS)


#define MRT_ROWS_SLAB1(P, RS, SIDE, TE, BX, BY, BZ, MASK)                                                             \
	"v_fma_f32 v51, " MRT_NEAR_##BX(RS, X, SIDE) ", " MRT_OP("ix", P) ", " MRT_OP("nrx", P) "\n"                      \
	"v_fma_f32 v52, " MRT_NEAR_##BY(RS, Y, SIDE) ", " MRT_OP("iy", P) ", " MRT_OP("nry", P) "\n"                      \
	"v_fma_f32 v53, " MRT_NEAR_##BZ(RS, Z, SIDE) ", " MRT_OP("iz", P) ", " MRT_OP("nrz", P) "\n"                      \
	"v_fma_f32 v54, " MRT_FAR_##BX(RS, X, SIDE) ", " MRT_OP("ix", P) ", " MRT_OP("nrx", P) "\n"                       \
	"v_fma_f32 v55, " MRT_FAR_##BY(RS, Y, SIDE) ", " MRT_OP("iy", P) ", " MRT_OP("nry", P) "\n"                       \
	"v_fma_f32 v57, " MRT_FAR_##BZ(RS, Z, SIDE) ", " MRT_OP("iz", P) ", " MRT_OP("nrz", P) "\n"                       \
	"v_max_f32 v53, v53, " MRT_OP("tmin", P) "\n"                                                                   \
	"v_min_f32 v57, v57, " MRT_OP("lim", P) "\n"                                                                    \
	"v_max3_f32 " TE ", v51, v52, v53\n"                                                                            \
	"v_min3_f32 v54, v54, v55, v57\n"                                                                               \
	"v_cmp_le_f32_e64 " MASK ", " TE ", v54\n"

#define MRT_ROWSC_CHILD(SIDE, TE, CULLBITS, MA, MB, BX, BY, BZ)                                                       \
	"s_and_b32 s48, s44, " CULLBITS "\n"                                 \
	"s_cbranch_scc1 L_cull" #SIDE "_%=\n"                                                                           \
	"s_cmp_eq_u64 s[60:61], 0\n"                                                                                    \
	"s_cbranch_scc1 L_" #SIDE "A0_%=\n"                                                                             \
	MRT_ROWS_SLAB1("A", RA, SIDE, TE, BX, BY, BZ, MA)                                                               \
	"L_" #SIDE "A1_%=:\n"                                                                                           \
	"s_cmp_eq_u64 s[62:63], 0\n"                                                                                    \
	"s_cbranch_scc1 L_" #SIDE "B0_%=\n"                                                                             \
	MRT_ROWS_SLAB1("B", RA, SIDE, TE, BX, BY, BZ, MB)                                                               \
	"L_" #SIDE "B1_%=:\n"
#define MRT_ROWSC_CHILD_OOL(SIDE, MA, MB)                                                                             \
	"L_cull" #SIDE "_%=:\n"                                                                                         \
	MRT_ROWSC_CNT_CULL                                                                                              \
	"s_mov_b64 " MA ", 0\n"                                                                                         \
	"s_mov_b64 " MB ", 0\n"                                                                                         \
	"s_branch L_" #SIDE "B1_%=\n"                                                                                   \
	"L_" #SIDE "A0_%=:\n"                                                                                           \
	"s_mov_b64 " MA ", 0\n"                                                                                         \
	"s_branch L_" #SIDE "A1_%=\n"                                                                                   \
	"L_" #SIDE "B0_%=:\n"                                                                                           \
	"s_mov_b64 " MB ", 0\n"                                                                                         \
	"s_branch L_" #SIDE "B1_%=\n"
#define MRT_ROWSC_CNT_CULL ""

#define MRT_ROWSC_VLOAD(VDST, REF)                                                                                   \
	"v_lshl_add_u32 v62, " REF ", 6, %[cvo]\n"                                                                      \
	"global_load_dword " VDST ", v62, %[rows]\n"

#ifndef MRT_ROWSC_KPF
#define MRT_ROWSC_KPF 0
#endif
#if MRT_ROWSC_KPF
#define MRT_ROWSC_KPREFETCH                                                                                           \
	"s_lshl_b32 s46, " RA_LREF ", 6\n"                                                                               \
	"s_lshl_b32 s47, " RA_RREF ", 6\n"                                                                               \
	"s_load_dword s64, %[rows], s46\n"                                                                              \
	"s_load_dword s65, %[rows], s47\n"
#else
#define MRT_ROWSC_KPREFETCH ""
#endif
#define MRT_ROWS_LOOPC(CNT_N, CNT_T, CNT_P, ANYA, ANYB, ANYDONE, BX, BY, BZ)                                          \
	asm volatile(                                                                                                   \
		"s_mov_b64 s[60:61], %[maskA]\n"                                                                            \
		"s_mov_b64 s[62:63], %[maskB]\n"                                                                            \
		"L_vload_%=:\n"                                     \
		MRT_ROWSC_VLOAD("v60", "%[curA]")                                                                           \
		"s_mov_b64 s[66:67], 0\n"                                                                                   \
		"L_loop_%=:\n"                                                                                              \
		"s_lshl_b32 s52, %[curA], 6\n"                                                                              \
		"s_load_dwordx16 s[20:35], %[rows], s52\n"                                                                  \
		"s_waitcnt lgkmcnt(0)\n"                                                                                    \
		"s_bitcmp1_b32 %[curA], 31\n"                                                                               \
		"s_cbranch_scc1 L_tri_%=\n"                                                                                 \
		CNT_N                                                                                                       \
		"s_waitcnt vmcnt(0)\n"                      \
		"v_cndmask_b32_e64 v58, v60, v61, s[66:67]\n"                                                               \
		"v_mul_f32 v58, v58, %[cw]\n"                                                                               \
		MRT_ROWSC_VLOAD("v60", RA_LREF)            \
		"v_add_f32_dpp v59, v58, v58 row_shr:1 row_mask:0xf bank_mask:0xf bound_ctrl:1\n"  \
		MRT_ROWSC_VLOAD("v61", RA_RREF)                                                                             \
		"v_add_f32_dpp v58, v59, v59 row_shr:2 row_mask:0xf bank_mask:0xf bound_ctrl:1\n"                           \
		"s_nop 1\n"                                                                                                 \
		"v_add_f32_dpp v59, v58, v58 row_shr:4 row_mask:0xf bank_mask:0xf bound_ctrl:1\n"                           \
		"v_cmp_lt_f32_e64 s[44:45], v59, %[ccc]\n"  \
		MRT_ROWSC_KPREFETCH                                                                                         \
		"s_or_b32 s44, s44, s45\n"                                                                                  \
		MRT_ROWSC_CHILD(L, "v50", "0x00800080", "s[36:37]", "s[40:41]", BX, BY, BZ)                                 \
		MRT_ROWSC_CHILD(R, "v56", "0x80008000", "s[38:39]", "s[42:43]", BX, BY, BZ)                                 \
		"s_or_b64 s[44:45], s[36:37], s[40:41]\n"                     \
		"s_cbranch_scc0 L_lmiss_%=\n"                                                                               \
		"s_or_b64 vcc, s[38:39], s[42:43]\n"                                              \
		"s_cbranch_scc0 L_onlyl_%=\n"                                                                               \
		      \
		"v_cmp_lt_f32_e64 s[46:47], v50, v56\n"                                           \
		"s_bitcmp1_b32 s46, 0\n"                                                                                    \
		"s_cselect_b32 s53, " RA_RREF ", " RA_LREF "\n"                                                   \
		"s_cselect_b32 %[curA], " RA_LREF ", " RA_RREF "\n"                                               \
		"s_cselect_b64 s[50:51], s[38:39], s[36:37]\n"                 \
		"s_cselect_b64 s[58:59], s[42:43], s[40:41]\n"                                                              \
		"s_cselect_b64 s[60:61], s[36:37], s[38:39]\n"                                        \
		"s_cselect_b64 s[62:63], s[40:41], s[42:43]\n"                                                              \
		"s_cselect_b64 s[66:67], 0, -1\n"                       \
		"v_mov_b32 v50, s50\n"                                                                                      \
		"v_mov_b32 v51, s51\n"                                                                                      \
		"v_mov_b32 v52, s58\n"                                                                                      \
		"v_mov_b32 v53, s59\n"                                                                                      \
		"v_mov_b32 v54, s53\n"                                                                                      \
		"ds_write_b128 %[spA], v[50:53]\n"                                                                          \
		"ds_write_b32 %[spA], v54 offset:16\n"                                                                      \
		"v_add_u32 %[spA], 32, %[spA]\n"                                                                            \
		CNT_P                                                                                                       \
		"s_branch L_loop_%=\n"                                                                                      \
		"L_onlyl_%=:\n"                                                                                             \
		"s_mov_b32 %[curA], " RA_LREF "\n"                                                                          \
		"s_mov_b64 s[60:61], s[36:37]\n"                                                                            \
		"s_mov_b64 s[62:63], s[40:41]\n"                                                                            \
		"s_mov_b64 s[66:67], 0\n"                                                                                   \
		"s_branch L_loop_%=\n"                                                                                      \
		"L_lmiss_%=:\n"                                                                                             \
		"s_or_b64 vcc, s[38:39], s[42:43]\n"                                                                        \
		"s_cbranch_scc0 L_pop_%=\n"                                                                                 \
		"s_mov_b32 %[curA], " RA_RREF "\n"                                                                          \
		"s_mov_b64 s[60:61], s[38:39]\n"                                                                            \
		"s_mov_b64 s[62:63], s[42:43]\n"                                                                            \
		"s_mov_b64 s[66:67], -1\n"                                                                                  \
		"s_branch L_loop_%=\n"                                                                                      \
		"L_tri_%=:\n"                                                                                               \
		CNT_T                                                                                                       \
		"s_cmp_eq_u64 s[60:61], 0\n"                                                                                \
		"s_cbranch_scc1 L_Atnext_%=\n"                                                                              \
		MRT_ROWS_TRI_TEST("A", RA, "s[60:61]", "%[curA]", ANYA)                                                     \
		"s_cmp_eq_u64 s[62:63], 0\n"                                                                                \
		"s_cbranch_scc1 L_Btnext_%=\n"                                                                              \
		MRT_ROWS_TRI_TEST("B", RA, "s[62:63]", "%[curA]", ANYB)                                                     \
		ANYDONE                                                                                                     \
		"s_bitcmp1_b32 " RA_FLAGS ", 0\n"                                       \
		"s_cbranch_scc1 L_pop_%=\n"                                                                                 \
		"s_add_u32 %[curA], %[curA], 1\n"                                                                           \
		"s_branch L_loop_%=\n"                                                                                      \
		"L_pop_%=:\n"                                                                                               \
		"v_add_u32 %[spA], -32, %[spA]\n"                                                                           \
		"ds_read_b128 v[50:53], %[spA]\n"                                                                           \
		"ds_read_b32 v54, %[spA] offset:16\n"                                                                       \
		"s_waitcnt lgkmcnt(0)\n"                                                                                    \
		"v_readfirstlane_b32 %[curA], v54\n"                                                                        \
		"v_readfirstlane_b32 s60, v50\n"                                                                            \
		"v_readfirstlane_b32 s61, v51\n"                                                                            \
		"v_readfirstlane_b32 s62, v52\n"                                                                            \
		"v_readfirstlane_b32 s63, v53\n"                                                                            \
		"s_cmp_lg_u32 %[curA], 0x7fffffff\n"                                                                        \
		"s_cbranch_scc1 L_vload_%=\n"                                                                               \
		"s_branch L_exit_%=\n"                                                                                      \
		MRT_ROWSC_CHILD_OOL(L, "s[36:37]", "s[40:41]")                                                              \
		MRT_ROWSC_CHILD_OOL(R, "s[38:39]", "s[42:43]")                                                              \
		"L_exit_%=:\n"                                                                                              \
		"s_waitcnt vmcnt(0)\n"                 \
		"s_mov_b64 %[maskA], s[60:61]\n"                                                                            \
		"s_mov_b64 %[maskB], s[62:63]\n"                                                                            \
		: MRT_ROWS_OUT(A, a), [limB] "+v"(b.lim), [btB] "+v"(b.bt), [buB] "+v"(b.bu), [bvB] "+v"(b.bv),             \
		  [bsB] "+v"(b.bs), [biB] "+v"(b.bi), [maskB] "+s"(b.mask), [cntn] "+s"(cnt_n), [cntt] "+s"(cnt_t), [cntp] "+s"(sp_max) \
		: MRT_ROWS_IN(A, a), MRT_ROWS_IN(B, b), [rows] "s"(rows), [qmask] "s"(qmask),                                \
		  [eps] "s"(eps), [vneg] "v"(vneg), [cw] "v"(cull.w), [ccc] "v"(cull.cc), [cvo] "v"(cull.voff)               \
		: MRT_ROWS_CLOBBERS, "v61", "v62")

struct CullRegs {
	float w;
	float cc;
	uint32_t voff;
};

#define MRT_ROWS_T_PRE "s_memtime s[64:65]\n s_waitcnt lgkmcnt(0)\n"
#define MRT_ROWS_T_POST "s_memtime s[66:67]\n s_waitcnt lgkmcnt(0)\n s_sub_u32 s64, s66, s64\n s_add_u32 %[cntw], %[cntw], s64\n"
#define MRT_ROWS_CNT_N "s_add_u32 %[cntn], %[cntn], 1\n"
#define MRT_ROWS_CNT_P "v_readfirstlane_b32 s52, %[spA]\n s_max_u32 %[cntp], %[cntp], s52\n"
#define MRT_ROWS_CNT_T "s_add_u32 %[cntt], %[cntt], 1\n"

__device__ __forceinline__ void rows_uniform(PacketRegs &s)
{
	s.cur = __builtin_amdgcn_readfirstlane(s.cur);
	const uint32_t lo = __builtin_amdgcn_readfirstlane((uint32_t)s.mask), hi = __builtin_amdgcn_readfirstlane((uint32_t)(s.mask >> 32));
	s.mask = ((unsigned long long)hi << 32) | lo;
}

template <int OCT, bool ANY_HIT, bool COUNT>
__device__ __forceinline__ void rows_walk_one(const float4 *rows, uint32_t qmask, PacketRegs &a, uint32_t &cnt_n, uint32_t &cnt_t, uint32_t &cnt_w, uint32_t &sp_max)
{
	const float eps = 1e-8f, vneg = -FLT_MAX;
	uint32_t ev = 0u;
#define MRT_W1(O, BX, BY, BZ)                                                                                         \
	if (OCT == O) {                                                                                                 \
		if (COUNT) { if (ANY_HIT) MRT_ROWS_LOOP1(MRT_ROWS_CNT_N, MRT_ROWS_CNT_T, MRT_ROWS_CNT_P, MRT_ROWS_T_PRE, MRT_ROWS_T_POST, MRT_ROWS_ANYHIT("A", "4"), BX, BY, BZ); \
			else MRT_ROWS_LOOP1(MRT_ROWS_CNT_N, MRT_ROWS_CNT_T, MRT_ROWS_CNT_P, MRT_ROWS_T_PRE, MRT_ROWS_T_POST, MRT_ROWS_NEAREST("A"), BX, BY, BZ); } \
		else { if (ANY_HIT) MRT_ROWS_LOOP1("", "", "", "", "", MRT_ROWS_ANYHIT("A", "4"), BX, BY, BZ);              \
			else MRT_ROWS_LOOP1("", "", "", "", "", MRT_ROWS_NEAREST("A"), BX, BY, BZ); }                           \
	}
	MRT_W1(0, 0, 0, 0) MRT_W1(1, 1, 0, 0) MRT_W1(2, 0, 1, 0) MRT_W1(3, 1, 1, 0) MRT_W1(4, 0, 0, 1) MRT_W1(5, 1, 0, 1) MRT_W1(6, 0, 1, 1) MRT_W1(7, 1, 1, 1)
#undef MRT_W1
	rows_uniform(a);
	cnt_n = __builtin_amdgcn_readfirstlane(cnt_n); cnt_t = __builtin_amdgcn_readfirstlane(cnt_t); cnt_w = __builtin_amdgcn_readfirstlane(cnt_w);
	sp_max = __builtin_amdgcn_readfirstlane(sp_max);
}

template <int OCT, bool ANY_HIT, bool COUNT>
__device__ __forceinline__ void rows_walk_wide(const float4 *rows, uint32_t qmask, PacketRegs &a, PacketRegs &b, uint32_t &cnt_n, uint32_t &cnt_t, uint32_t &sp_max)
{
	const float eps = 1e-8f, vneg = -FLT_MAX;
#define MRT_WW(O, BX, BY, BZ)                                                                                         \
	if (OCT == O) {                                                                                                 \
		if (COUNT) { if (ANY_HIT) MRT_ROWS_LOOPW(MRT_ROWS_CNT_N, MRT_ROWS_CNT_T, MRT_ROWS_CNT_P, MRT_ROWSW_ANYHIT("A"), MRT_ROWSW_ANYHIT("B"), MRT_ROWSW_ANYDONE, BX, BY, BZ); \
			else MRT_ROWS_LOOPW(MRT_ROWS_CNT_N, MRT_ROWS_CNT_T, MRT_ROWS_CNT_P, MRT_ROWS_NEAREST("A"), MRT_ROWS_NEAREST("B"), "", BX, BY, BZ); } \
		else { if (ANY_HIT) MRT_ROWS_LOOPW("", "", "", MRT_ROWSW_ANYHIT("A"), MRT_ROWSW_ANYHIT("B"), MRT_ROWSW_ANYDONE, BX, BY, BZ); \
			else MRT_ROWS_LOOPW("", "", "", MRT_ROWS_NEAREST("A"), MRT_ROWS_NEAREST("B"), "", BX, BY, BZ); }        \
	}
	MRT_WW(0, 0, 0, 0) MRT_WW(1, 1, 0, 0) MRT_WW(2, 0, 1, 0) MRT_WW(3, 1, 1, 0) MRT_WW(4, 0, 0, 1) MRT_WW(5, 1, 0, 1) MRT_WW(6, 0, 1, 1) MRT_WW(7, 1, 1, 1)
#undef MRT_WW
	rows_uniform(a);
	cnt_n = __builtin_amdgcn_readfirstlane(cnt_n); cnt_t = __builtin_amdgcn_readfirstlane(cnt_t);
	sp_max = __builtin_amdgcn_readfirstlane(sp_max);
}

template <int OCT, bool ANY_HIT, bool COUNT>
__device__ __forceinline__ void rows_walk_cull(const float4 *rows, uint32_t qmask, PacketRegs &a, PacketRegs &b, const CullRegs &cull, uint32_t &cnt_n, uint32_t &cnt_t, uint32_t &sp_max)
{
	const float eps = 1e-8f, vneg = -FLT_MAX;
#define MRT_WC(O, BX, BY, BZ)                                                                                         \
	if (OCT == O) {                                                                                                 \
		if (COUNT) { if (ANY_HIT) MRT_ROWS_LOOPC(MRT_ROWS_CNT_N, MRT_ROWS_CNT_T, MRT_ROWS_CNT_P, MRT_ROWSW_ANYHIT("A"), MRT_ROWSW_ANYHIT("B"), MRT_ROWSW_ANYDONE, BX, BY, BZ); \
			else MRT_ROWS_LOOPC(MRT_ROWS_CNT_N, MRT_ROWS_CNT_T, MRT_ROWS_CNT_P, MRT_ROWS_NEAREST("A"), MRT_ROWS_NEAREST("B"), "", BX, BY, BZ); } \
		else { if (ANY_HIT) MRT_ROWS_LOOPC("", "", "", MRT_ROWSW_ANYHIT("A"), MRT_ROWSW_ANYHIT("B"), MRT_ROWSW_ANYDONE, BX, BY, BZ); \
			else MRT_ROWS_LOOPC("", "", "", MRT_ROWS_NEAREST("A"), MRT_ROWS_NEAREST("B"), "", BX, BY, BZ); }        \
	}
	MRT_WC(0, 0, 0, 0) MRT_WC(1, 1, 0, 0) MRT_WC(2, 0, 1, 0) MRT_WC(3, 1, 1, 0) MRT_WC(4, 0, 0, 1) MRT_WC(5, 1, 0, 1) MRT_WC(6, 0, 1, 1) MRT_WC(7, 1, 1, 1)
#undef MRT_WC
	rows_uniform(a);
	cnt_n = __builtin_amdgcn_readfirstlane(cnt_n); cnt_t = __builtin_amdgcn_readfirstlane(cnt_t);
	sp_max = __builtin_amdgcn_readfirstlane(sp_max);
}

__device__ __forceinline__ CullRegs cull_setup(const RayRegs &ra, const RayRegs &rb, bool valid_a, bool valid_b, unsigned long long part_a,
		unsigned long long part_b, float scene_abs_max, uint32_t lane)
{
	CullRegs c;
	c.w = 0.0f; c.cc = -__builtin_inff(); c.voff = (lane & 15u) * 4u;
	const bool corners = (part_a & 1ull) && (part_a >> 56 & 1ull) && (part_b >> 7 & 1ull) && (part_b >> 63 & 1ull);
	if (!corners) return c;
#define MRT_RL(v, l) __builtin_bit_cast(float, __builtin_amdgcn_readlane(__builtin_bit_cast(int, v), l))
	const float ox = MRT_RL(ra.ox, 0), oy = MRT_RL(ra.oy, 0), oz = MRT_RL(ra.oz, 0);
	const float tl[3] = { MRT_RL(ra.dx, 0), MRT_RL(ra.dy, 0), MRT_RL(ra.dz, 0) }, bl[3] = { MRT_RL(ra.dx, 56), MRT_RL(ra.dy, 56), MRT_RL(ra.dz, 56) };
	const float tr[3] = { MRT_RL(rb.dx, 7), MRT_RL(rb.dy, 7), MRT_RL(rb.dz, 7) }, br[3] = { MRT_RL(rb.dx, 63), MRT_RL(rb.dy, 63), MRT_RL(rb.dz, 63) };
	float cen[3] = { tl[0] + tr[0] + bl[0] + br[0], tl[1] + tr[1] + bl[1] + br[1], tl[2] + tr[2] + bl[2] + br[2] };
	const float cl = __builtin_sqrtf(cen[0] * cen[0] + cen[1] * cen[1] + cen[2] * cen[2]);
	if (!(cl > 0.0f)) return c;
	cen[0] /= cl; cen[1] /= cl; cen[2] /= cl;
	const uint32_t k = lane >> 4;
	const float *pa = k == 0u ? tl : (k == 1u ? tr : (k == 2u ? br : bl)), *pb = k == 0u ? tr : (k == 1u ? br : (k == 2u ? bl : tl));
	float n[3] = { pa[1] * pb[2] - pa[2] * pb[1], pa[2] * pb[0] - pa[0] * pb[2], pa[0] * pb[1] - pa[1] * pb[0] };
	const float nl = __builtin_sqrtf(n[0] * n[0] + n[1] * n[1] + n[2] * n[2]);
	bool ok = nl > 0.0f;
	const float inv = ok ? 1.0f / nl : 0.0f;
	n[0] *= inv; n[1] *= inv; n[2] *= inv;
	if (n[0] * cen[0] + n[1] * cen[1] + n[2] * cen[2] < 0.0f) { n[0] = -n[0]; n[1] = -n[1]; n[2] = -n[2]; }
	const float push = 5e-5f;
	n[0] += push * cen[0]; n[1] += push * cen[1]; n[2] += push * cen[2];
	bool inside = true;
	for (int q = 0; q < 4; q++) {
		const float qx = MRT_RL(n[0], 16 * q), qy = MRT_RL(n[1], 16 * q), qz = MRT_RL(n[2], 16 * q);
		const float da = qx * ra.dx + qy * ra.dy + qz * ra.dz, la = __builtin_sqrtf(ra.dx * ra.dx + ra.dy * ra.dy + ra.dz * ra.dz);
		const float db = qx * rb.dx + qy * rb.dy + qz * rb.dz, lb = __builtin_sqrtf(rb.dx * rb.dx + rb.dy * rb.dy + rb.dz * rb.dz);
		if (valid_a && !(da >= 1e-5f * la)) inside = false;
		if (valid_b && !(db >= 1e-5f * lb)) inside = false;
	}
#undef MRT_RL
	if (valid_a && !(ra.ox == ox && ra.oy == oy && ra.oz == oz && ra.t_min >= 0.0f)) inside = false;
	if (valid_b && !(rb.ox == ox && rb.oy == oy && rb.oz == oz && rb.t_min >= 0.0f)) inside = false;
	ok = ok && __builtin_isfinite(n[0]) && __builtin_isfinite(n[1]) && __builtin_isfinite(n[2]);
	const bool planes_ok = (__ballot(ok) & 0x0001000100010001ull) == 0x0001000100010001ull;
	if (__ballot(!inside) != 0ull || !planes_ok) return c;
	const float n1 = __builtin_fabsf(n[0]) + __builtin_fabsf(n[1]) + __builtin_fabsf(n[2]);
	const float o1 = __builtin_fabsf(ox) + __builtin_fabsf(oy) + __builtin_fabsf(oz);
	const float err = 8.0f * 5.9604645e-8f * n1 * (scene_abs_max + o1);
	const float cc = (n[0] * ox + n[1] * oy + n[2] * oz) - err;
	if (__ballot(!__builtin_isfinite(cc)) != 0ull) return c;
	const uint32_t d = lane & 15u, axis = d & 3u;
	const bool is_max = (d >> 2 & 1u) != 0u;
	const float na = axis == 0u ? n[0] : (axis == 1u ? n[1] : n[2]);
	c.w = (axis < 3u && ((na >= 0.0f) == is_max)) ? na : 0.0f;
	c.cc = (d == 7u || d == 15u) ? cc : -__builtin_inff();
	return c;
}

__device__ __forceinline__ void rows_init(PacketRegs &s, const RayRegs &r, bool takes_part, uint32_t sp)
{
	s.ox = r.ox; s.oy = r.oy; s.oz = r.oz; s.dx = r.dx; s.dy = r.dy; s.dz = r.dz; s.tmin = r.t_min;
	s.ix = safe_inv(r.dx); s.iy = safe_inv(r.dy); s.iz = safe_inv(r.dz);
	s.nrx = -(r.ox * s.ix); s.nry = -(r.oy * s.iy); s.nrz = -(r.oz * s.iz);
	s.bt = r.t_max; s.bu = 0.0f; s.bv = 0.0f; s.bs = 0xFFFFFFFFu; s.bi = 0xFFFFFFFFu;
	s.lim = (!takes_part || r.t_min >= r.t_max) ? -FLT_MAX : r.t_max;
	s.sp = sp; s.cur = 0u; s.mask = 0ull;
}

__device__ __forceinline__ int rows_octant(const RayRegs &r, bool part, unsigned long long &part_mask)
{
	part_mask = __ballot(part);
	const unsigned long long sx = __ballot(part && safe_inv(r.dx) < 0.0f), sy = __ballot(part && safe_inv(r.dy) < 0.0f),
			sz = __ballot(part && safe_inv(r.dz) < 0.0f);
	const bool uniform = (sx == 0ull || sx == part_mask) && (sy == 0ull || sy == part_mask) && (sz == 0ull || sz == part_mask);
	return uniform ? ((sx ? 1 : 0) | (sy ? 2 : 0) | (sz ? 4 : 0)) : 8;
}

#ifndef MRT_ROWS_WPE
#define MRT_ROWS_WPE 8
#endif
template <bool ANY_HIT, bool COUNT, int PACKETS, int WG, bool CULL = false>
__global__ __launch_bounds__(WG) __attribute__((amdgpu_waves_per_eu(MRT_ROWS_WPE, 8))) void trace_packet_rows_kernel(const TraceParams p)
{
	__shared__ __attribute__((aligned(16))) uint32_t wave_stack[WG / MRT_WAVE][PACKETS][(MRT_PACKET_STACK + 1) * 4];
	if (skip_launch(p)) return;
	uint32_t block = blockIdx.x;
	if (p.xcd_swizzle) {
		const uint32_t per = gridDim.x >> 3;
		if (block < (per << 3)) block = (block & 7u) * per + (block >> 3);
	}
	const uint32_t wave = threadIdx.x / MRT_WAVE, lane = threadIdx.x & (MRT_WAVE - 1);
	const uint32_t wave_s = __builtin_amdgcn_readfirstlane(wave), block_s = block;
	const uint64_t g_a = (((uint64_t)block * (WG / MRT_WAVE) + wave) * PACKETS) * MRT_WAVE + lane, g_b = g_a + MRT_WAVE;
	uint64_t idx = 0; uint32_t px = 0, py = 0;
	const bool valid_a = lane_ray_index_g(p, g_a, idx, px, py);
	RayRegs ra = {0.0f, 0.0f, 0.0f, 0.0f, 0.0f, 0.0f, 1.0f, 0.0f}, rb = ra;
	if (valid_a) load_ray(p, idx, px, py, ra);
	bool valid_b = false;
	if (PACKETS == 2) {
		valid_b = lane_ray_index_g(p, g_b, idx, px, py);
		if (valid_b) load_ray(p, idx, px, py, rb);
	}
	if (__ballot(valid_a || valid_b) == 0ull) return;

	const float4 *rows = reinterpret_cast<const float4 *>(p.row_array);
	uint32_t *stack_a = wave_stack[wave][0], *stack_b = wave_stack[wave][PACKETS - 1];
	*(volatile uint32_t *)&stack_a[0] = kSentinel;
	if (PACKETS == 2) *(volatile uint32_t *)&stack_b[0] = kSentinel;
	PacketRegs A, B;
	rows_init(A, ra, valid_a, (uint32_t)(uintptr_t)(__attribute__((address_space(3))) uint32_t *)(stack_a + 4));
	rows_init(B, rb, valid_b, (uint32_t)(uintptr_t)(__attribute__((address_space(3))) uint32_t *)(stack_b + 4));

	unsigned long long part_a = 0ull, part_b = 0ull;
	const int oct_a = rows_octant(ra, valid_a, part_a);
	const int oct_b = PACKETS == 2 ? rows_octant(rb, valid_b, part_b) : 8;
	uint32_t cnt_n = 0u, cnt_t = 0u;
	uint32_t cnt_w = 0u;
	uint32_t sp_wide = 0u, sp_one = 0u;
	if (p.tile_cost != nullptr && lane == 0u) note_tile_start(p, g_a);
	if (COUNT) *(volatile unsigned long long *)&stack_a[2] = __builtin_amdgcn_s_memtime();
	bool done_a = part_a == 0ull, done_b = part_b == 0ull;
	if (PACKETS == 2 && !done_a && !done_b && oct_a == oct_b && oct_a != 8) {
		*(volatile uint32_t *)&stack_a[4] = kSentinel;
		A.sp += 16u;
		A.mask = part_a; B.mask = part_b;
		if (CULL) {
			const CullRegs cull = cull_setup(ra, rb, valid_a, valid_b, part_a, part_b, p.scene_abs_max, lane);
#define MRT_RWC(O) case O: rows_walk_cull<O, ANY_HIT, COUNT>(rows, p.query_mask, A, B, cull, cnt_n, cnt_t, sp_wide); break;
			switch (oct_a) { MRT_RWC(0) MRT_RWC(1) MRT_RWC(2) MRT_RWC(3) MRT_RWC(4) MRT_RWC(5) MRT_RWC(6) MRT_RWC(7) }
#undef MRT_RWC
		} else {
#define MRT_RW2(O) case O: rows_walk_wide<O, ANY_HIT, COUNT>(rows, p.query_mask, A, B, cnt_n, cnt_t, sp_wide); break;
		switch (oct_a) { MRT_RW2(0) MRT_RW2(1) MRT_RW2(2) MRT_RW2(3) MRT_RW2(4) MRT_RW2(5) MRT_RW2(6) MRT_RW2(7) }
#undef MRT_RW2
		}
		done_a = done_b = true;
	}
#define MRT_RW1(O, S) case O: rows_walk_one<O, ANY_HIT, COUNT>(rows, p.query_mask, S, cnt_n, cnt_t, cnt_w, sp_one); break;
	if (!done_a && oct_a != 8) { switch (oct_a) { MRT_RW1(0, A) MRT_RW1(1, A) MRT_RW1(2, A) MRT_RW1(3, A) MRT_RW1(4, A) MRT_RW1(5, A) MRT_RW1(6, A) MRT_RW1(7, A) } done_a = true; }
	if (PACKETS == 2 && !done_b && oct_b != 8) { switch (oct_b) { MRT_RW1(0, B) MRT_RW1(1, B) MRT_RW1(2, B) MRT_RW1(3, B) MRT_RW1(4, B) MRT_RW1(5, B) MRT_RW1(6, B) MRT_RW1(7, B) } done_b = true; }
#undef MRT_RW1
	uint32_t slot_a = A.bs == 0xFFFFFFFFu ? 0xFFFFFFFFu : A.bs - p.n_nodes, slot_b = B.bs == 0xFFFFFFFFu ? 0xFFFFFFFFu : B.bs - p.n_nodes;
	if (!done_a) {
		uint32_t nn = 0, nt = 0, nd = 0;
		A.bt = ra.t_max;
		packet_traverse<8, ANY_HIT, COUNT>(p, ra, stack_a, A.bt, A.bu, A.bv, slot_a, nn, nt, nd, 0u, 0u, nullptr, !valid_a);
		if (COUNT) { cnt_n += __builtin_amdgcn_readfirstlane(nn); cnt_t += __builtin_amdgcn_readfirstlane(nt); }
	}
	if (PACKETS == 2 && !done_b) {
		uint32_t nn = 0, nt = 0, nd = 0;
		B.bt = rb.t_max;
		packet_traverse<8, ANY_HIT, COUNT>(p, rb, stack_b, B.bt, B.bu, B.bv, slot_b, nn, nt, nd, 0u, 0u, nullptr, !valid_b);
		if (COUNT) { cnt_n += __builtin_amdgcn_readfirstlane(nn); cnt_t += __builtin_amdgcn_readfirstlane(nt); }
	}

	{
		const uint32_t lane2 = __builtin_amdgcn_mbcnt_hi(~0u, __builtin_amdgcn_mbcnt_lo(~0u, 0u));
		const uint64_t h_a = (((uint64_t)block_s * (WG / MRT_WAVE) + wave_s) * PACKETS) * MRT_WAVE + lane2;
		uint64_t idx2 = 0; uint32_t px2 = 0, py2 = 0;
		if (lane_ray_index_g(p, h_a, idx2, px2, py2)) finish_ray(p, idx2, ra, A.bt, A.bu, A.bv, slot_a);
		if (PACKETS == 2 && lane_ray_index_g(p, h_a + MRT_WAVE, idx2, px2, py2)) finish_ray(p, idx2, rb, B.bt, B.bu, B.bv, slot_b);
		if (p.tile_cost != nullptr && lane2 == 0u) note_tile_cost(p, h_a);
	}
	const unsigned long long t_start = COUNT ? *(volatile unsigned long long *)&stack_a[2] : 0ull;
	if (COUNT && lane == 0u && (p.count_mode != 2u || (blockIdx.x & 15u) == 0u)) {
		atomicAdd(&p.counters[kCntFetchWaitCycles], (unsigned long long)cnt_w);
		atomicAdd(&p.counters[kCntWaveCycles], __builtin_amdgcn_s_memtime() - t_start);
		atomicAdd(&p.counters[kCntWaves], 1ull);
	}
	if (COUNT && p.count_mode != 2u) {
		const uint32_t base = (uint32_t)(uintptr_t)(__attribute__((address_space(3))) uint32_t *)stack_a;
		const uint32_t e_wide = sp_wide > base ? (sp_wide - base) / 32u : 0u, e_one = sp_one > base ? ((sp_one - base) % 1040u) / 16u : 0u;
		atomicMax(&p.counters[kCntMaxStack], (unsigned long long)(e_wide > e_one ? e_wide : e_one));
	}
	if (COUNT && p.count_mode != 2u) {
		if (valid_a) packet_count(p, cnt_n, cnt_t, 0u, slot_a != 0xFFFFFFFFu, part_a | part_b);
		if (PACKETS == 2 && valid_b) { atomicAdd(&p.counters[kCntRays], 1ull); if (slot_b != 0xFFFFFFFFu) atomicAdd(&p.counters[kCntHits], 1ull); }
	}
}
```

Measured before the change: 8731.

## Add resident-ray child prefetch variant to culled rows traversal loop

Adds a KPF template parameter to the culled dual-packet rows kernel, selected when culling is on and the input is not a grid. In that case the inline-asm cull loop issues a scalar prefetch of child node rows before the slab tests. The cull loop assembly is also restructured into shared DECIDE, TRI_STEP and POP macros with separate left and right loop entry labels, so node loads for the chosen child can be overlapped. This aims to hide scalar memory latency on the traversal critical path, at the cost of extra scalar loads and more complex hand-written control flow.

```diff
diff --git a/messyerraytracer_amd/csrc/kernels.hip b/messyerraytracer_amd/csrc/kernels.hip
--- a/messyerraytracer_amd/csrc/kernels.hip
+++ b/messyerraytracer_amd/csrc/kernels.hip
@@ -634,6 +634,9 @@
 	va_list ap; va_start(ap, fmt); vsnprintf(g_variant, sizeof(g_variant), fmt, ap); va_end(ap);
 }
 #define MRT_B(x) ((x) ? "true" : "false")
+#ifndef MRT_ROWSC_KPF_RESIDENT
+#define MRT_ROWSC_KPF_RESIDENT 1
+#endif
 #ifndef MRT_ROWS_WG_LARGE
 #define MRT_ROWS_WG_LARGE MRT_WG
 #endif
@@ -686,19 +689,27 @@
 		const uint32_t rows_wg = packets == 2u && p.rows_wg == 64u ? 64u : (packets == 2u ? (uint32_t)MRT_ROWS_WG_LARGE : (uint32_t)MRT_WG);
 		const uint64_t rblocks = (threads + packets * rows_wg - 1) / (packets * rows_wg);
 		dim3 rgrid((uint32_t)rblocks), rwg(rows_wg);
-#define MRT_LAUNCH_ROWS(A, C, N, W, F) hipLaunchKernelGGL((trace_packet_rows_kernel<A, C, N, W, F>), rgrid, rwg, p.extra_lds, stream, p)
-#define MRT_LAUNCH_ROWS_AC(N, W, F)                                                                                    \
+#define MRT_LAUNCH_ROWS(A, C, N, W, F, K) hipLaunchKernelGGL((trace_packet_rows_kernel<A, C, N, W, F, K>), rgrid, rwg, p.extra_lds, stream, p)
+#define MRT_LAUNCH_ROWS_AC(N, W, F, K)                                                                                 \
 		do {                                                                                                        \
-			if (count) { if (any_hit) MRT_LAUNCH_ROWS(true, true, N, W, F); else MRT_LAUNCH_ROWS(false, true, N, W, F); } \
-			else { if (any_hit) MRT_LAUNCH_ROWS(true, false, N, W, F); else MRT_LAUNCH_ROWS(false, false, N, W, F); }   \
+			if (count) { if (any_hit) MRT_LAUNCH_ROWS(true, true, N, W, F, K); else MRT_LAUNCH_ROWS(false, true, N, W, F, K); } \
+			else { if (any_hit) MRT_LAUNCH_ROWS(true, false, N, W, F, K); else MRT_LAUNCH_ROWS(false, false, N, W, F, K); }   \
+		} while (0)
+#define MRT_LAUNCH_ROWS_CULL(W)                                                                                        \
+		do {                                                                                                        \
+			if (!cull) MRT_LAUNCH_ROWS_AC(2, W, false, false);                                                      \
+			else if (kpf) MRT_LAUNCH_ROWS_AC(2, W, true, true);                                                     \
+			else MRT_LAUNCH_ROWS_AC(2, W, true, false);                                                             \
 		} while (0)
 		const bool cull = packets == 2u && (p.rows_cull == 1u || (p.rows_cull == 2u && p.in_fmt == IN_GRID));
-		if (packets == 2u && rows_wg == 64u) { if (cull) MRT_LAUNCH_ROWS_AC(2, 64, true); else MRT_LAUNCH_ROWS_AC(2, 64, false); }
-		else if (packets == 2u) { if (cull) MRT_LAUNCH_ROWS_AC(2, MRT_ROWS_WG_LARGE, true); else MRT_LAUNCH_ROWS_AC(2, MRT_ROWS_WG_LARGE, false); }
-		else MRT_LAUNCH_ROWS_AC(1, MRT_WG, false);
+		const bool kpf = cull && p.in_fmt != IN_GRID && MRT_ROWSC_KPF_RESIDENT;
+		if (packets == 2u && rows_wg == 64u) MRT_LAUNCH_ROWS_CULL(64);
+		else if (packets == 2u) MRT_LAUNCH_ROWS_CULL(MRT_ROWS_WG_LARGE);
+		else MRT_LAUNCH_ROWS_AC(1, MRT_WG, false, false);
+#undef MRT_LAUNCH_ROWS_CULL
 #undef MRT_LAUNCH_ROWS_AC
 #undef MRT_LAUNCH_ROWS
-		note_variant("trace_packet_rows_kernel<%s, %s, %u, %u, %s>", MRT_B(any_hit), MRT_B(count), packets, rows_wg, MRT_B(cull));
+		note_variant("trace_packet_rows_kernel<%s, %s, %u, %u, %s, %s>", MRT_B(any_hit), MRT_B(count), packets, rows_wg, MRT_B(cull), MRT_B(kpf));
 		return hipGetLastError();
 	}
 	if ((p.kernel == MRT_KERNEL_PACKET_ASM || p.kernel == MRT_KERNEL_PACKET_DUAL || p.kernel == MRT_KERNEL_PACKET_ROWS || p.kernel == MRT_KERNEL_PACKET_QUAD) && p.n_nodes < kAsmNodeLimit) {
diff --git a/messyerraytracer_amd/csrc/packet_rows_kernel.h b/messyerraytracer_amd/csrc/packet_rows_kernel.h
--- a/messyerraytracer_amd/csrc/packet_rows_kernel.h
+++ b/messyerraytracer_amd/csrc/packet_rows_kernel.h
@@ -311,94 +311,103 @@
 	"global_load_dword v60, v55, %[rows]\n"
 #endif
 
-#define MRT_ROWS_LOOPW(CNT_N, CNT_T, CNT_P, ANYA, ANYB, ANYDONE, BX, BY, BZ)                                                 \
-	asm volatile(                                                                                                   \
-		"s_mov_b64 s[60:61], %[maskA]\n"                                                                            \
-		"s_mov_b64 s[62:63], %[maskB]\n"                                                                            \
-		"L_loop_%=:\n"                                                                                              \
-		"s_lshl_b32 s52, %[curA], 6\n"                                                                              \
-		"s_load_dwordx16 s[20:35], %[rows], s52\n"                                                                  \
-		"s_waitcnt lgkmcnt(0)\n"                                                                                    \
-		"s_bitcmp1_b32 %[curA], 31\n"                                                                               \
-		"s_cbranch_scc1 L_tri_%=\n"                                                                                 \
-		CNT_N                                                                                                       \
-		MRT_ROWSW_KPREFETCH                                                                                         \
-		MRT_ROWSW_GROUP_SLAB("A", "s[60:61]", "s[36:37]", "s[38:39]", BX, BY, BZ)                                   \
-		MRT_ROWSW_GROUP_SLAB("B", "s[62:63]", "s[40:41]", "s[42:43]", BX, BY, BZ)                                   \
-		"s_or_b64 s[44:45], s[36:37], s[40:41]\n"                     \
-		"s_cbranch_scc0 L_lmiss_%=\n"                                                                               \
-		"s_or_b64 vcc, s[38:39], s[42:43]\n"                                              \
-		"s_cbranch_scc0 L_onlyl_%=\n"                                                                               \
-		      \
-		"v_cmp_lt_f32_e64 s[46:47], v50, v56\n"                                           \
-		"s_bitcmp1_b32 s46, 0\n"                                                                                    \
-		"s_cselect_b32 s53, " RA_RREF ", " RA_LREF "\n"                                                   \
-		"s_cselect_b32 %[curA], " RA_LREF ", " RA_RREF "\n"                                               \
-		"s_cselect_b64 s[50:51], s[38:39], s[36:37]\n"                 \
-		"s_cselect_b64 s[58:59], s[42:43], s[40:41]\n"                                                              \
-		"s_cselect_b64 s[60:61], s[36:37], s[38:39]\n"                                        \
-		"s_cselect_b64 s[62:63], s[40:41], s[42:43]\n"                                                              \
-		"v_mov_b32 v50, s50\n"                                                                                      \
-		"v_mov_b32 v51, s51\n"                                                                                      \
-		"v_mov_b32 v52, s58\n"                                                                                      \
-		"v_mov_b32 v53, s59\n"                                                                                      \
-		"v_mov_b32 v54, s53\n"                                                                                      \
-		"ds_write_b128 %[spA], v[50:53]\n"                                                                          \
-		"ds_write_b32 %[spA], v54 offset:16\n"                                                                      \
-		"v_add_u32 %[spA], 32, %[spA]\n"                                                                            \
-		CNT_P                                                                                                       \
-		MRT_ROWSW_FARPREFETCH                                                                                       \
-		"s_branch L_loop_%=\n"                                                                                      \
-		"L_onlyl_%=:\n"                                                                                             \
-		"s_mov_b32 %[curA], " RA_LREF "\n"                                                                          \
-		"s_mov_b64 s[60:61], s[36:37]\n"                                                                            \
-		"s_mov_b64 s[62:63], s[40:41]\n"                                                                            \
-		"s_branch L_loop_%=\n"                                                                                      \
-		"L_lmiss_%=:\n"                                                                                             \
-		"s_or_b64 vcc, s[38:39], s[42:43]\n"                                                                        \
-		"s_cbranch_scc0 L_pop_%=\n"                                                                                 \
-		"s_mov_b32 %[curA], " RA_RREF "\n"                                                                          \
-		"s_mov_b64 s[60:61], s[38:39]\n"                                                                            \
-		"s_mov_b64 s[62:63], s[42:43]\n"                                                                            \
-		"s_branch L_loop_%=\n"                                                                                      \
-		"L_tri_%=:\n"                                                                                               \
-		CNT_T                                                                                                       \
-		"s_cmp_eq_u64 s[60:61], 0\n"                                                                                \
-		"s_cbranch_scc1 L_Atnext_%=\n"                                                                              \
-		MRT_ROWS_TRI_TEST("A", RA, "s[60:61]", "%[curA]", ANYA)                                                     \
-		"s_cmp_eq_u64 s[62:63], 0\n"                                                                                \
-		"s_cbranch_scc1 L_Btnext_%=\n"                                                                              \
-		MRT_ROWS_TRI_TEST("B", RA, "s[62:63]", "%[curA]", ANYB)                                                     \
-		ANYDONE                                                                                                     \
-		"s_bitcmp1_b32 " RA_FLAGS ", 0\n"                                       \
-		"s_cbranch_scc1 L_pop_%=\n"                                                                                 \
-		"s_add_u32 %[curA], %[curA], 1\n"                                                                           \
-		"s_branch L_loop_%=\n"                                                                                      \
-		"L_pop_%=:\n"                                                                                               \
-		"v_add_u32 %[spA], -32, %[spA]\n"                                                                           \
-		"ds_read_b128 v[50:53], %[spA]\n"                                                                           \
-		"ds_read_b32 v54, %[spA] offset:16\n"                                                                       \
-		"s_waitcnt lgkmcnt(0)\n"                                                                                    \
-		"v_readfirstlane_b32 %[curA], v54\n"                                                                        \
-		"v_readfirstlane_b32 s60, v50\n"                                                                            \
-		"v_readfirstlane_b32 s61, v51\n"                                                                            \
-		"v_readfirstlane_b32 s62, v52\n"                                                                            \
-		"v_readfirstlane_b32 s63, v53\n"                                                                            \
-		"s_cmp_lg_u32 %[curA], 0x7fffffff\n"                                                                        \
-		"s_cbranch_scc1 L_loop_%=\n"                                                                                \
-		"s_branch L_exit_%=\n"                                                                                      \
-		MRT_ROWSW_GROUP_SKIP("A", "s[36:37]", "s[38:39]")                                                           \
-		MRT_ROWSW_GROUP_SKIP("B", "s[40:41]", "s[42:43]")                                                           \
-		"L_exit_%=:\n"                                                                                              \
-		"s_waitcnt vmcnt(0)\n"                    \
-		"s_mov_b64 %[maskA], s[60:61]\n"                                                                            \
-		"s_mov_b64 %[maskB], s[62:63]\n"                                                                            \
-		: MRT_ROWS_OUT(A, a), [limB] "+v"(b.lim), [btB] "+v"(b.bt), [buB] "+v"(b.bu), [bvB] "+v"(b.bv),             \
+#define MRT_ROWSW_DECIDE(CNT_P, BOTH_TAIL, LEFT_NEXT, RIGHT_NEXT)                                                     \
+	"s_or_b64 s[44:45], s[36:37], s[40:41]\n"                           \
+	"s_cbranch_scc0 L_lmiss_%=\n"                                                                                     \
+	"s_or_b64 vcc, s[38:39], s[42:43]\n"                                                    \
+	"s_cbranch_scc0 L_onlyl_%=\n"                                                                                     \
+	            \
+	"v_cmp_lt_f32_e64 s[46:47], v50, v56\n"                                                 \
+	"s_bitcmp1_b32 s46, 0\n"                                                                                          \
+	"s_cselect_b32 s53, " RA_RREF ", " RA_LREF "\n"                                                         \
+	"s_cselect_b32 %[curA], " RA_LREF ", " RA_RREF "\n"                                                     \
+	"s_cselect_b64 s[50:51], s[38:39], s[36:37]\n"                       \
+	"s_cselect_b64 s[58:59], s[42:43], s[40:41]\n"                                                                    \
+	"s_cselect_b64 s[60:61], s[36:37], s[38:39]\n"                                              \
+	"s_cselect_b64 s[62:63], s[40:41], s[42:43]\n"                                                                    \
+	"v_mov_b32 v50, s50\n"                                                                                            \
+	"v_mov_b32 v51, s51\n"                                                                                            \
+	"v_mov_b32 v52, s58\n"                                                                                            \
+	"v_mov_b32 v53, s59\n"                                                                                            \
+	"v_mov_b32 v54, s53\n"                                                                                            \
+	"ds_write_b128 %[spA], v[50:53]\n"                                                                                \
+	"ds_write_b32 %[spA], v54 offset:16\n"                                                                            \
+	"v_add_u32 %[spA], 32, %[spA]\n"                                                                                  \
+	CNT_P                                                                                                             \
+	BOTH_TAIL                                                                                                         \
+	"L_onlyl_%=:\n"                                                                                                   \
+	"s_mov_b32 %[curA], " RA_LREF "\n"                                                                                \
+	"s_mov_b64 s[60:61], s[36:37]\n"                                                                                  \
+	"s_mov_b64 s[62:63], s[40:41]\n"                                                                                  \
+	"s_branch " LEFT_NEXT "\n"                                                                                        \
+	"L_lmiss_%=:\n"                                                                                                   \
+	"s_or_b64 vcc, s[38:39], s[42:43]\n"                                                                              \
+	"s_cbranch_scc0 L_pop_%=\n"                                                                                       \
+	"s_mov_b32 %[curA], " RA_RREF "\n"                                                                                \
+	"s_mov_b64 s[60:61], s[38:39]\n"                                                                                  \
+	"s_mov_b64 s[62:63], s[42:43]\n"                                                                                  \
+	"s_branch " RIGHT_NEXT "\n"
+#define MRT_ROWSW_TRI_STEP(CNT_T, ANYA, ANYB, ANYDONE)                                                                \
+	"L_tri_%=:\n"                                                                                                     \
+	CNT_T                                                                                                             \
+	"s_cmp_eq_u64 s[60:61], 0\n"                                                                                      \
+	"s_cbranch_scc1 L_Atnext_%=\n"                                                                                    \
+	MRT_ROWS_TRI_TEST("A", RA, "s[60:61]", "%[curA]", ANYA)                                                           \
+	"s_cmp_eq_u64 s[62:63], 0\n"                                                                                      \
+	"s_cbranch_scc1 L_Btnext_%=\n"                                                                                    \
+	MRT_ROWS_TRI_TEST("B", RA, "s[62:63]", "%[curA]", ANYB)                                                           \
+	ANYDONE                                                                                                           \
+	"s_bitcmp1_b32 " RA_FLAGS ", 0\n"                                             \
+	"s_cbranch_scc1 L_pop_%=\n"                                                                                       \
+	"s_add_u32 %[curA], %[curA], 1\n"                                                                                 \
+	"s_branch L_loop_%=\n"
+#define MRT_ROWSW_POP(NEXT)                                                                                           \
+	"L_pop_%=:\n"                                                                                                     \
+	"v_add_u32 %[spA], -32, %[spA]\n"                                                                                 \
+	"ds_read_b128 v[50:53], %[spA]\n"                                                                                 \
+	"ds_read_b32 v54, %[spA] offset:16\n"                                                                             \
+	"s_waitcnt lgkmcnt(0)\n"                                                                                          \
+	"v_readfirstlane_b32 %[curA], v54\n"                                                                              \
+	"v_readfirstlane_b32 s60, v50\n"                                                                                  \
+	"v_readfirstlane_b32 s61, v51\n"                                                                                  \
+	"v_readfirstlane_b32 s62, v52\n"                                                                                  \
+	"v_readfirstlane_b32 s63, v53\n"                                                                                  \
+	"s_cmp_lg_u32 %[curA], 0x7fffffff\n"                                                                              \
+	"s_cbranch_scc1 " NEXT "\n"                                                                                       \
+	"s_branch L_exit_%=\n"
+
+#define MRT_ROWS_LOOPW(CNT_N, CNT_T, CNT_P, ANYA, ANYB, ANYDONE, BX, BY, BZ)                                          \
+	asm volatile(                                                                                                     \
+		"s_mov_b64 s[60:61], %[maskA]\n"                                                                              \
+		"s_mov_b64 s[62:63], %[maskB]\n"                                                                              \
+		"L_loop_%=:\n"                                                                                                \
+		"s_lshl_b32 s52, %[curA], 6\n"                                                                                \
+		"s_load_dwordx16 s[20:35], %[rows], s52\n"                                                                    \
+		"s_waitcnt lgkmcnt(0)\n"                                                                                      \
+		"s_bitcmp1_b32 %[curA], 31\n"                                                                                 \
+		"s_cbranch_scc1 L_tri_%=\n"                                                                                   \
+		CNT_N                                                                                                         \
+		MRT_ROWSW_KPREFETCH                                                                                           \
+		MRT_ROWSW_GROUP_SLAB("A", "s[60:61]", "s[36:37]", "s[38:39]", BX, BY, BZ)                                     \
+		MRT_ROWSW_GROUP_SLAB("B", "s[62:63]", "s[40:41]", "s[42:43]", BX, BY, BZ)                                     \
+		MRT_ROWSW_DECIDE(CNT_P, MRT_ROWSW_FARPREFETCH "s_branch L_loop_%=\n", "L_loop_%=", "L_loop_%=")               \
+		MRT_ROWSW_TRI_STEP(CNT_T, ANYA, ANYB, ANYDONE)                                                                \
+		MRT_ROWSW_POP("L_loop_%=")                                                                                    \
+		MRT_ROWSW_GROUP_SKIP("A", "s[36:37]", "s[38:39]")                                                             \
+		MRT_ROWSW_GROUP_SKIP("B", "s[40:41]", "s[42:43]")                                                             \
+		"L_exit_%=:\n"                                                                                                \
+		"s_waitcnt vmcnt(0)\n"                       \
+		"s_mov_b64 %[maskA], s[60:61]\n"                                                                              \
+		"s_mov_b64 %[maskB], s[62:63]\n"                                                                              \
+		: MRT_ROWS_OUT(A, a), [limB] "+v"(b.lim), [btB] "+v"(b.bt), [buB] "+v"(b.bu), [bvB] "+v"(b.bv),               \
 		  [bsB] "+v"(b.bs), [biB] "+v"(b.bi), [maskB] "+s"(b.mask), [cntn] "+s"(cnt_n), [cntt] "+s"(cnt_t), [cntp] "+s"(sp_max) \
 		: MRT_ROWS_IN(A, a), MRT_ROWS_IN(B, b), [rows] "s"(rows), [qmask] "s"(qmask), [eps] "s"(eps), [vneg] "v"(vneg) \
 		: MRT_ROWS_CLOBBERS)
 
 
+#ifndef MRT_ROWSC_VMCNT_L
+#define MRT_ROWSC_VMCNT_L "1"
+#endif
 #define MRT_ROWS_SLAB1(P, RS, SIDE, TE, BX, BY, BZ, MASK)                                                             \
 	"v_fma_f32 v51, " MRT_NEAR_##BX(RS, X, SIDE) ", " MRT_OP("ix", P) ", " MRT_OP("nrx", P) "\n"                      \
 	"v_fma_f32 v52, " MRT_NEAR_##BY(RS, Y, SIDE) ", " MRT_OP("iy", P) ", " MRT_OP("nry", P) "\n"                      \
@@ -406,155 +415,85 @@
 	"v_fma_f32 v54, " MRT_FAR_##BX(RS, X, SIDE) ", " MRT_OP("ix", P) ", " MRT_OP("nrx", P) "\n"                       \
 	"v_fma_f32 v55, " MRT_FAR_##BY(RS, Y, SIDE) ", " MRT_OP("iy", P) ", " MRT_OP("nry", P) "\n"                       \
 	"v_fma_f32 v57, " MRT_FAR_##BZ(RS, Z, SIDE) ", " MRT_OP("iz", P) ", " MRT_OP("nrz", P) "\n"                       \
-	"v_max_f32 v53, v53, " MRT_OP("tmin", P) "\n"                                                                   \
-	"v_min_f32 v57, v57, " MRT_OP("lim", P) "\n"                                                                    \
-	"v_max3_f32 " TE ", v51, v52, v53\n"                                                                            \
-	"v_min3_f32 v54, v54, v55, v57\n"                                                                               \
+	"v_max_f32 v53, v53, " MRT_OP("tmin", P) "\n"                                                                     \
+	"v_min_f32 v57, v57, " MRT_OP("lim", P) "\n"                                                                      \
+	"v_max3_f32 " TE ", v51, v52, v53\n"                                                                              \
+	"v_min3_f32 v54, v54, v55, v57\n"                                                                                 \
 	"v_cmp_le_f32_e64 " MASK ", " TE ", v54\n"
 
-#define MRT_ROWSC_CHILD(SIDE, TE, CULLBITS, MA, MB, BX, BY, BZ)                                                       \
-	"s_and_b32 s48, s44, " CULLBITS "\n"                                 \
-	"s_cbranch_scc1 L_cull" #SIDE "_%=\n"                                                                           \
-	"s_cmp_eq_u64 s[60:61], 0\n"                                                                                    \
-	"s_cbranch_scc1 L_" #SIDE "A0_%=\n"                                                                             \
-	MRT_ROWS_SLAB1("A", RA, SIDE, TE, BX, BY, BZ, MA)                                                               \
-	"L_" #SIDE "A1_%=:\n"                                                                                           \
-	"s_cmp_eq_u64 s[62:63], 0\n"                                                                                    \
-	"s_cbranch_scc1 L_" #SIDE "B0_%=\n"                                                                             \
-	MRT_ROWS_SLAB1("B", RA, SIDE, TE, BX, BY, BZ, MB)                                                               \
-	"L_" #SIDE "B1_%=:\n"
-#define MRT_ROWSC_CHILD_OOL(SIDE, MA, MB)                                                                             \
-	"L_cull" #SIDE "_%=:\n"                                                                                         \
-	MRT_ROWSC_CNT_CULL                                                                                              \
-	"s_mov_b64 " MA ", 0\n"                                                                                         \
-	"s_mov_b64 " MB ", 0\n"                                                                                         \
-	"s_branch L_" #SIDE "B1_%=\n"                                                                                   \
-	"L_" #SIDE "A0_%=:\n"                                                                                           \
-	"s_mov_b64 " MA ", 0\n"                                                                                         \
-	"s_branch L_" #SIDE "A1_%=\n"                                                                                   \
-	"L_" #SIDE "B0_%=:\n"                                                                                           \
-	"s_mov_b64 " MB ", 0\n"                                                                                         \
-	"s_branch L_" #SIDE "B1_%=\n"
-#define MRT_ROWSC_CNT_CULL ""
-
-#define MRT_ROWSC_VLOAD(VDST, REF)                                                                                   \
-	"v_lshl_add_u32 v62, " REF ", 6, %[cvo]\n"                                                                      \
+#define MRT_ROWSC_ONE_CHILD(SIDE, REF, NEXT, BX, BY, BZ)                                                              \
+	"s_cmp_eq_u64 s[60:61], 0\n"                                                                                      \
+	"s_cbranch_scc1 L_" #SIDE "oA_%=\n"                                                                               \
+	MRT_ROWS_SLAB1("A", RA, SIDE, "v50", BX, BY, BZ, "s[60:61]")                                                      \
+	"L_" #SIDE "oA_%=:\n"                                                                                             \
+	"s_cmp_eq_u64 s[62:63], 0\n"                                                                                      \
+	"s_cbranch_scc1 L_" #SIDE "oB_%=\n"                                                                               \
+	MRT_ROWS_SLAB1("B", RA, SIDE, "v50", BX, BY, BZ, "s[62:63]")                                                      \
+	"L_" #SIDE "oB_%=:\n"                                                                                             \
+	"s_or_b64 vcc, s[60:61], s[62:63]\n"                                                                              \
+	"s_cbranch_scc0 L_pop_%=\n"                                                                                       \
+	"s_mov_b32 %[curA], " REF "\n"                                                                                    \
+	"s_branch " NEXT "\n"
+
+#define MRT_ROWSC_VLOAD(VDST, REF)                                                                                    \
+	"v_lshl_add_u32 v62, " REF ", 6, %[cvo]\n"                                                                        \
 	"global_load_dword " VDST ", v62, %[rows]\n"
 
-#ifndef MRT_ROWSC_KPF
-#define MRT_ROWSC_KPF 0
-#endif
-#if MRT_ROWSC_KPF
-#define MRT_ROWSC_KPREFETCH                                                                                           \
-	"s_lshl_b32 s46, " RA_LREF ", 6\n"                                                                               \
-	"s_lshl_b32 s47, " RA_RREF ", 6\n"                                                                               \
-	"s_load_dword s64, %[rows], s46\n"                                                                              \
-	"s_load_dword s65, %[rows], s47\n"
-#else
-#define MRT_ROWSC_KPREFETCH ""
-#endif
-#define MRT_ROWS_LOOPC(CNT_N, CNT_T, CNT_P, ANYA, ANYB, ANYDONE, BX, BY, BZ)                                          \
-	asm volatile(                                                                                                   \
-		"s_mov_b64 s[60:61], %[maskA]\n"                                                                            \
-		"s_mov_b64 s[62:63], %[maskB]\n"                                                                            \
-		"L_vload_%=:\n"                                     \
-		MRT_ROWSC_VLOAD("v60", "%[curA]")                                                                           \
-		"s_mov_b64 s[66:67], 0\n"                                                                                   \
-		"L_loop_%=:\n"                                                                                              \
-		"s_lshl_b32 s52, %[curA], 6\n"                                                                              \
-		"s_load_dwordx16 s[20:35], %[rows], s52\n"                                                                  \
-		"s_waitcnt lgkmcnt(0)\n"                                                                                    \
-		"s_bitcmp1_b32 %[curA], 31\n"                                                                               \
-		"s_cbranch_scc1 L_tri_%=\n"                                                                                 \
-		CNT_N                                                                                                       \
-		"s_waitcnt vmcnt(0)\n"                      \
-		"v_cndmask_b32_e64 v58, v60, v61, s[66:67]\n"                                                               \
-		"v_mul_f32 v58, v58, %[cw]\n"                                                                               \
+#define MRT_ROWSC_HEAD(CNT_N, VM, VSRC)                                                                               \
+	"s_lshl_b32 s52, %[curA], 6\n"                                                                                    \
+	"s_load_dwordx16 s[20:35], %[rows], s52\n"                                                                        \
+	"s_waitcnt lgkmcnt(0)\n"                                                                                          \
+	"s_bitcmp1_b32 %[curA], 31\n"                                                                                     \
+	"s_cbranch_scc1 L_tri_%=\n"                                                                                       \
+	CNT_N                                                                                                             \
+	"s_waitcnt vmcnt(" VM ")\n"                                                                                       \
+	"v_mul_f32 v58, " VSRC ", %[cw]\n"
+
+#define MRT_ROWS_LOOPC(CNT_N, CNT_T, CNT_P, ANYA, ANYB, ANYDONE, KPF, BX, BY, BZ)                                     \
+	asm volatile(                                                                                                     \
+		"s_mov_b64 s[60:61], %[maskA]\n"                                                                              \
+		"s_mov_b64 s[62:63], %[maskB]\n"                                                                              \
+		"L_vload_%=:\n"                                      \
+		MRT_ROWSC_VLOAD("v61", "%[curA]")                                                                             \
+		"L_loop_%=:\n"                                     \
+		MRT_ROWSC_HEAD(CNT_N, "0", "v61")                                                                             \
+		"s_branch L_node_%=\n"                                                                                        \
+		"L_loopl_%=:\n"                                                                \
+		MRT_ROWSC_HEAD(CNT_N, MRT_ROWSC_VMCNT_L, "v60")                                                               \
+		"L_node_%=:\n"                                                                                                \
 		MRT_ROWSC_VLOAD("v60", RA_LREF)            \
 		"v_add_f32_dpp v59, v58, v58 row_shr:1 row_mask:0xf bank_mask:0xf bound_ctrl:1\n"  \
-		MRT_ROWSC_VLOAD("v61", RA_RREF)                                                                             \
-		"v_add_f32_dpp v58, v59, v59 row_shr:2 row_mask:0xf bank_mask:0xf bound_ctrl:1\n"                           \
-		"s_nop 1\n"                                                                                                 \
-		"v_add_f32_dpp v59, v58, v58 row_shr:4 row_mask:0xf bank_mask:0xf bound_ctrl:1\n"                           \
-		"v_cmp_lt_f32_e64 s[44:45], v59, %[ccc]\n"  \
-		MRT_ROWSC_KPREFETCH                                                                                         \
-		"s_or_b32 s44, s44, s45\n"                                                                                  \
-		MRT_ROWSC_CHILD(L, "v50", "0x00800080", "s[36:37]", "s[40:41]", BX, BY, BZ)                                 \
-		MRT_ROWSC_CHILD(R, "v56", "0x80008000", "s[38:39]", "s[42:43]", BX, BY, BZ)                                 \
-		"s_or_b64 s[44:45], s[36:37], s[40:41]\n"                     \
-		"s_cbranch_scc0 L_lmiss_%=\n"                                                                               \
-		"s_or_b64 vcc, s[38:39], s[42:43]\n"                                              \
-		"s_cbranch_scc0 L_onlyl_%=\n"                                                                               \
-		      \
-		"v_cmp_lt_f32_e64 s[46:47], v50, v56\n"                                           \
-		"s_bitcmp1_b32 s46, 0\n"                                                                                    \
-		"s_cselect_b32 s53, " RA_RREF ", " RA_LREF "\n"                                                   \
-		"s_cselect_b32 %[curA], " RA_LREF ", " RA_RREF "\n"                                               \
-		"s_cselect_b64 s[50:51], s[38:39], s[36:37]\n"                 \
-		"s_cselect_b64 s[58:59], s[42:43], s[40:41]\n"                                                              \
-		"s_cselect_b64 s[60:61], s[36:37], s[38:39]\n"                                        \
-		"s_cselect_b64 s[62:63], s[40:41], s[42:43]\n"                                                              \
-		"s_cselect_b64 s[66:67], 0, -1\n"                       \
-		"v_mov_b32 v50, s50\n"                                                                                      \
-		"v_mov_b32 v51, s51\n"                                                                                      \
-		"v_mov_b32 v52, s58\n"                                                                                      \
-		"v_mov_b32 v53, s59\n"                                                                                      \
-		"v_mov_b32 v54, s53\n"                                                                                      \
-		"ds_write_b128 %[spA], v[50:53]\n"                                                                          \
-		"ds_write_b32 %[spA], v54 offset:16\n"                                                                      \
-		"v_add_u32 %[spA], 32, %[spA]\n"                                                                            \
-		CNT_P                                                                                                       \
-		"s_branch L_loop_%=\n"                                                                                      \
-		"L_onlyl_%=:\n"                                                                                             \
-		"s_mov_b32 %[curA], " RA_LREF "\n"                                                                          \
-		"s_mov_b64 s[60:61], s[36:37]\n"                                                                            \
-		"s_mov_b64 s[62:63], s[40:41]\n"                                                                            \
-		"s_mov_b64 s[66:67], 0\n"                                                                                   \
-		"s_branch L_loop_%=\n"                                                                                      \
-		"L_lmiss_%=:\n"                                                                                             \
-		"s_or_b64 vcc, s[38:39], s[42:43]\n"                                                                        \
-		"s_cbranch_scc0 L_pop_%=\n"                                                                                 \
-		"s_mov_b32 %[curA], " RA_RREF "\n"                                                                          \
-		"s_mov_b64 s[60:61], s[38:39]\n"                                                                            \
-		"s_mov_b64 s[62:63], s[42:43]\n"                                                                            \
-		"s_mov_b64 s[66:67], -1\n"                                                                                  \
-		"s_branch L_loop_%=\n"                                                                                      \
-		"L_tri_%=:\n"                                                                                               \
-		CNT_T                                                                                                       \
-		"s_cmp_eq_u64 s[60:61], 0\n"                                                                                \
-		"s_cbranch_scc1 L_Atnext_%=\n"                                                                              \
-		MRT_ROWS_TRI_TEST("A", RA, "s[60:61]", "%[curA]", ANYA)                                                     \
-		"s_cmp_eq_u64 s[62:63], 0\n"                                                                                \
-		"s_cbranch_scc1 L_Btnext_%=\n"                                                                              \
-		MRT_ROWS_TRI_TEST("B", RA, "s[62:63]", "%[curA]", ANYB)                                                     \
-		ANYDONE                                                                                                     \
-		"s_bitcmp1_b32 " RA_FLAGS ", 0\n"                                       \
-		"s_cbranch_scc1 L_pop_%=\n"                                                                                 \
-		"s_add_u32 %[curA], %[curA], 1\n"                                                                           \
-		"s_branch L_loop_%=\n"                                                                                      \
-		"L_pop_%=:\n"                                                                                               \
-		"v_add_u32 %[spA], -32, %[spA]\n"                                                                           \
-		"ds_read_b128 v[50:53], %[spA]\n"                                                                           \
-		"ds_read_b32 v54, %[spA] offset:16\n"                                                                       \
-		"s_waitcnt lgkmcnt(0)\n"                                                                                    \
-		"v_readfirstlane_b32 %[curA], v54\n"                                                                        \
-		"v_readfirstlane_b32 s60, v50\n"                                                                            \
-		"v_readfirstlane_b32 s61, v51\n"                                                                            \
-		"v_readfirstlane_b32 s62, v52\n"                                                                            \
-		"v_readfirstlane_b32 s63, v53\n"                                                                            \
-		"s_cmp_lg_u32 %[curA], 0x7fffffff\n"                                                                        \
-		"s_cbranch_scc1 L_vload_%=\n"                                                                               \
-		"s_branch L_exit_%=\n"                                                                                      \
-		MRT_ROWSC_CHILD_OOL(L, "s[36:37]", "s[40:41]")                                                              \
-		MRT_ROWSC_CHILD_OOL(R, "s[38:39]", "s[42:43]")                                                              \
-		"L_exit_%=:\n"                                                                                              \
-		"s_waitcnt vmcnt(0)\n"                 \
-		"s_mov_b64 %[maskA], s[60:61]\n"                                                                            \
-		"s_mov_b64 %[maskB], s[62:63]\n"                                                                            \
-		: MRT_ROWS_OUT(A, a), [limB] "+v"(b.lim), [btB] "+v"(b.bt), [buB] "+v"(b.bu), [bvB] "+v"(b.bv),             \
+		MRT_ROWSC_VLOAD("v61", RA_RREF)                                                                               \
+		"v_add_f32_dpp v58, v59, v59 row_shr:2 row_mask:0xf bank_mask:0xf bound_ctrl:1\n"                             \
+		"s_nop 1\n"                                                                                                   \
+		"v_add_f32_dpp v59, v58, v58 row_shr:4 row_mask:0xf bank_mask:0xf bound_ctrl:1\n"                             \
+		"v_cmp_lt_f32_e64 vcc, v59, %[ccc]\n"      \
+		KPF                                                                                                           \
+		"s_cbranch_vccnz L_some_%=\n"              \
+		MRT_ROWSW_GROUP_SLAB("A", "s[60:61]", "s[36:37]", "s[38:39]", BX, BY, BZ)                                     \
+		MRT_ROWSW_GROUP_SLAB("B", "s[62:63]", "s[40:41]", "s[42:43]", BX, BY, BZ)                                     \
+		MRT_ROWSW_DECIDE(CNT_P, "s_cbranch_scc1 L_loopl_%=\n s_branch L_loop_%=\n", "L_loopl_%=", "L_loop_%=")        \
+		MRT_ROWSW_TRI_STEP(CNT_T, ANYA, ANYB, ANYDONE)                                                                \
+		MRT_ROWSW_POP("L_vload_%=")                                                                                   \
+		"L_some_%=:\n"                                                                                                \
+		"s_or_b32 s44, vcc_lo, vcc_hi\n"                                                                              \
+		"s_and_b32 s48, s44, 0x00800080\n"                            \
+		"s_cbranch_scc0 L_lonly_%=\n"                                                     \
+		"s_and_b32 s48, s44, 0x80008000\n"                                                                            \
+		"s_cbranch_scc1 L_pop_%=\n"                                                                         \
+		MRT_ROWSC_ONE_CHILD(R, RA_RREF, "L_loop_%=", BX, BY, BZ)                                                      \
+		"L_lonly_%=:\n"                                                                                               \
+		MRT_ROWSC_ONE_CHILD(L, RA_LREF, "L_loopl_%=", BX, BY, BZ)                                                     \
+		MRT_ROWSW_GROUP_SKIP("A", "s[36:37]", "s[38:39]")                                                             \
+		MRT_ROWSW_GROUP_SKIP("B", "s[40:41]", "s[42:43]")                                                             \
+		"L_exit_%=:\n"                                                                                                \
+		"s_waitcnt vmcnt(0)\n"                   \
+		"s_mov_b64 %[maskA], s[60:61]\n"                                                                              \
+		"s_mov_b64 %[maskB], s[62:63]\n"                                                                              \
+		: MRT_ROWS_OUT(A, a), [limB] "+v"(b.lim), [btB] "+v"(b.bt), [buB] "+v"(b.bu), [bvB] "+v"(b.bv),               \
 		  [bsB] "+v"(b.bs), [biB] "+v"(b.bi), [maskB] "+s"(b.mask), [cntn] "+s"(cnt_n), [cntt] "+s"(cnt_t), [cntp] "+s"(sp_max) \
-		: MRT_ROWS_IN(A, a), MRT_ROWS_IN(B, b), [rows] "s"(rows), [qmask] "s"(qmask),                                \
-		  [eps] "s"(eps), [vneg] "v"(vneg), [cw] "v"(cull.w), [ccc] "v"(cull.cc), [cvo] "v"(cull.voff)               \
+		: MRT_ROWS_IN(A, a), MRT_ROWS_IN(B, b), [rows] "s"(rows), [qmask] "s"(qmask),                                 \
+		  [eps] "s"(eps), [vneg] "v"(vneg), [cw] "v"(cull.w), [ccc] "v"(cull.cc), [cvo] "v"(cull.voff)                \
 		: MRT_ROWS_CLOBBERS, "v61", "v62")
 
 struct CullRegs {
@@ -568,6 +507,7 @@
 #define MRT_ROWS_CNT_N "s_add_u32 %[cntn], %[cntn], 1\n"
 #define MRT_ROWS_CNT_P "v_readfirstlane_b32 s52, %[spA]\n s_max_u32 %[cntp], %[cntp], s52\n"
 #define MRT_ROWS_CNT_T "s_add_u32 %[cntt], %[cntt], 1\n"
+#define MRT_ROWSC_CNT_P MRT_ROWS_CNT_P "s_bitcmp1_b32 s46, 0\n"
 
 __device__ __forceinline__ void rows_uniform(PacketRegs &s)
 {
@@ -613,19 +553,22 @@
 	sp_max = __builtin_amdgcn_readfirstlane(sp_max);
 }
 
-template <int OCT, bool ANY_HIT, bool COUNT>
+template <int OCT, bool ANY_HIT, bool COUNT, bool KPF>
 __device__ __forceinline__ void rows_walk_cull(const float4 *rows, uint32_t qmask, PacketRegs &a, PacketRegs &b, const CullRegs &cull, uint32_t &cnt_n, uint32_t &cnt_t, uint32_t &sp_max)
 {
 	const float eps = 1e-8f, vneg = -FLT_MAX;
+#define MRT_WC2(K, BX, BY, BZ)                                                                                        \
+	do {                                                                                                            \
+		if (COUNT) { if (ANY_HIT) MRT_ROWS_LOOPC(MRT_ROWS_CNT_N, MRT_ROWS_CNT_T, MRT_ROWSC_CNT_P, MRT_ROWSW_ANYHIT("A"), MRT_ROWSW_ANYHIT("B"), MRT_ROWSW_ANYDONE, K, BX, BY, BZ); \
+			else MRT_ROWS_LOOPC(MRT_ROWS_CNT_N, MRT_ROWS_CNT_T, MRT_ROWSC_CNT_P, MRT_ROWS_NEAREST("A"), MRT_ROWS_NEAREST("B"), "", K, BX, BY, BZ); } \
+		else { if (ANY_HIT) MRT_ROWS_LOOPC("", "", "", MRT_ROWSW_ANYHIT("A"), MRT_ROWSW_ANYHIT("B"), MRT_ROWSW_ANYDONE, K, BX, BY, BZ); \
+			else MRT_ROWS_LOOPC("", "", "", MRT_ROWS_NEAREST("A"), MRT_ROWS_NEAREST("B"), "", K, BX, BY, BZ); }     \
+	} while (0)
 #define MRT_WC(O, BX, BY, BZ)                                                                                         \
-	if (OCT == O) {                                                                                                 \
-		if (COUNT) { if (ANY_HIT) MRT_ROWS_LOOPC(MRT_ROWS_CNT_N, MRT_ROWS_CNT_T, MRT_ROWS_CNT_P, MRT_ROWSW_ANYHIT("A"), MRT_ROWSW_ANYHIT("B"), MRT_ROWSW_ANYDONE, BX, BY, BZ); \
-			else MRT_ROWS_LOOPC(MRT_ROWS_CNT_N, MRT_ROWS_CNT_T, MRT_ROWS_CNT_P, MRT_ROWS_NEAREST("A"), MRT_ROWS_NEAREST("B"), "", BX, BY, BZ); } \
-		else { if (ANY_HIT) MRT_ROWS_LOOPC("", "", "", MRT_ROWSW_ANYHIT("A"), MRT_ROWSW_ANYHIT("B"), MRT_ROWSW_ANYDONE, BX, BY, BZ); \
-			else MRT_ROWS_LOOPC("", "", "", MRT_ROWS_NEAREST("A"), MRT_ROWS_NEAREST("B"), "", BX, BY, BZ); }        \
-	}
+	if (OCT == O) { if (KPF) MRT_WC2(MRT_ROWSW_KPREFETCH, BX, BY, BZ); else MRT_WC2("", BX, BY, BZ); }
 	MRT_WC(0, 0, 0, 0) MRT_WC(1, 1, 0, 0) MRT_WC(2, 0, 1, 0) MRT_WC(3, 1, 1, 0) MRT_WC(4, 0, 0, 1) MRT_WC(5, 1, 0, 1) MRT_WC(6, 0, 1, 1) MRT_WC(7, 1, 1, 1)
 #undef MRT_WC
+#undef MRT_WC2
 	rows_uniform(a);
 	cnt_n = __builtin_amdgcn_readfirstlane(cnt_n); cnt_t = __builtin_amdgcn_readfirstlane(cnt_t);
 	sp_max = __builtin_amdgcn_readfirstlane(sp_max);
@@ -705,7 +648,7 @@
 #ifndef MRT_ROWS_WPE
 #define MRT_ROWS_WPE 8
 #endif
-template <bool ANY_HIT, bool COUNT, int PACKETS, int WG, bool CULL = false>
+template <bool ANY_HIT, bool COUNT, int PACKETS, int WG, bool CULL = false, bool KPF = false>
 __global__ __launch_bounds__(WG) __attribute__((amdgpu_waves_per_eu(MRT_ROWS_WPE, 8))) void trace_packet_rows_kernel(const TraceParams p)
 {
 	__shared__ __attribute__((aligned(16))) uint32_t wave_stack[WG / MRT_WAVE][PACKETS][(MRT_PACKET_STACK + 1) * 4];
@@ -752,7 +695,7 @@
 		A.mask = part_a; B.mask = part_b;
 		if (CULL) {
 			const CullRegs cull = cull_setup(ra, rb, valid_a, valid_b, part_a, part_b, p.scene_abs_max, lane);
-#define MRT_RWC(O) case O: rows_walk_cull<O, ANY_HIT, COUNT>(rows, p.query_mask, A, B, cull, cnt_n, cnt_t, sp_wide); break;
+#define MRT_RWC(O) case O: rows_walk_cull<O, ANY_HIT, COUNT, KPF>(rows, p.query_mask, A, B, cull, cnt_n, cnt_t, sp_wide); break;
 			switch (oct_a) { MRT_RWC(0) MRT_RWC(1) MRT_RWC(2) MRT_RWC(3) MRT_RWC(4) MRT_RWC(5) MRT_RWC(6) MRT_RWC(7) }
 #undef MRT_RWC
 		} else {
```

Measured after the change: 8616. -1.3%, worse.
